# RayforceDB/rayforce

Hardware: AMD Instinct MI355X
Metric: rows/s on filter→group-by→sum, 1e9-row i64/f64; % HBM roofline at 1/2/4/8 GPU (higher is better)
Workload: dtype f64

## Files before the change

### include/rfx_hip.h

```cpp
#ifndef RFX_HIP_H
#define RFX_HIP_H

#ifndef __HIPCC_RTC__
#include <stddef.h>
#endif
#include <stdint.h>

#ifdef __cplusplus
extern "C" {
#endif
#ifndef __HIPCC_RTC__
#pragma GCC visibility push(default)
#endif

enum {
    RFX_OK = 0,
    RFX_ENODEV = -1,
    RFX_EINVAL = -2,
    RFX_ENOMEM = -3,
    RFX_EHIP = -4,
    RFX_ELIMIT = -5,
    RFX_ESTATE = -6
};

// ... 53 lines not shown
typedef struct rfx_xnode {
    int32_t op;
    int32_t _pad;
    rfx_xoperand_t l, r;
} rfx_xnode_t;

typedef struct rfx_agg {
    const void *d_col;
    int32_t col_type;
    int32_t kind;
    int32_t xop;
    int32_t xflags;
    const void *d_xrhs_col;
    int32_t xrhs_type;
    int32_t nxnodes;
    union {
        int64_t xrhs_i;
        double xrhs_f;
    };
    const rfx_xnode_t *xnodes;
} rfx_agg_t;
int rfx_agg_input_type(const rfx_agg_t *a);

typedef struct rfx_partial {
    int64_t isum;
    double fsum;
    int64_t cnt;
    int64_t ext;
    int64_t pos;
    int64_t _rsv[3];
} rfx_partial_t;

typedef struct rfx_value {
    int32_t type;
    int32_t is_null;
    union {
        int64_t i;
        double f;
    };
} rfx_value_t;

typedef struct rfx_ctx rfx_ctx_t;

int rfx_hip_device_count(void);
const char *rfx_hip_last_error(void);
const char *rfx_hip_version(void);
#define RFX_STREAM_LEGACY ((void *)(uintptr_t)1)
int rfx_hip_ctx_create(int device, void *stream, rfx_ctx_t **out);
int rfx_hip_ctx_destroy(rfx_ctx_t *ctx);
int rfx_hip_ctx_sync(rfx_ctx_t *ctx);
int rfx_hip_ctx_set_stream(rfx_ctx_t *ctx, void *stream);
enum {
    RFX_TUNE_NO_LDS_TABLES = 1,
    RFX_TUNE_NO_PARTITION = 2,
    RFX_TUNE_NO_BIG_LDS = 4,
    RFX_TUNE_PART_3WG = 8,
    RFX_TUNE_NO_WRITE_COMBINE = 16,
    RFX_TUNE_DIRECT_WC = 32,
    RFX_TUNE_FUSED_KEYS = 64,
    RFX_TUNE_NO_FUSED_SCOPE = 128,
    RFX_TUNE_NO_SOA_WC = 2048,
    RFX_TUNE_NO_LDS_SPLIT = 1024,
    RFX_TUNE_NO_EMIT_WC = 512,
    RFX_TUNE_NO_SEL_COMPACT = 256,
    RFX_TUNE_NO_DEEP_GROUP = 4096,
    RFX_TUNE_NO_LDS_REPLICAS = 8192,
    RFX_TUNE_NO_CHUNK = 16384,
    RFX_TUNE_CHUNK_SMALL = 32768,
    RFX_TUNE_CHUNK_CONTIG = 65536,
    RFX_TUNE_CHUNK_QUEUE = 131072,
    RFX_TUNE_CHUNK_BINS = 262144,
    RFX_TUNE_NO_RTC = 524288,
    RFX_TUNE_NO_PLANE = 1048576,
    RFX_TUNE_NO_WHERE_ONCE = 2097152
};
int rfx_hip_ctx_tune(rfx_ctx_t *ctx, int blocks_per_cu, int flags);
enum {
    RFX_STAT_PLANE_SCATTER = 0,
    RFX_STAT_PLANE_FALLBACK = 1,
    RFX_STAT_PLANE_AGGREGATE = 2,
    RFX_STAT_CHUNK_SCATTER = 3,
    RFX_STAT_CHUNK_AGGREGATE = 4,
    RFX_STAT_MASK_PASSES = 5,
    RFX_STAT_WHERE_ONCE = 6
};
int64_t rfx_hip_ctx_stat(rfx_ctx_t *ctx, int which);

int rfx_hip_malloc(rfx_ctx_t *ctx, void **d_ptr, size_t bytes);
int rfx_hip_free(rfx_ctx_t *ctx, void *d_ptr);
int rfx_hip_ctx_trim(rfx_ctx_t *ctx);
int rfx_hip_h2d(rfx_ctx_t *ctx, void *d_dst, const void *src, size_t bytes);
int rfx_hip_d2h(rfx_ctx_t *ctx, void *dst, const void *d_src, size_t bytes);
int rfx_hip_d2h_async(rfx_ctx_t *ctx, void *dst, const void *d_src, size_t bytes);
int rfx_hip_memset(rfx_ctx_t *ctx, void *d_dst, int byte, size_t bytes);
int rfx_hip_fill_i64(rfx_ctx_t *ctx, int64_t *d_dst, int64_t n, int64_t value);
void rfx_hip_rtc_stats(int64_t *launches, int64_t *compiles);
void rfx_hip_rtc_cache_stats(int64_t *loaded_from_disk, int64_t *written_to_disk);
int rfx_hip_rtc_prewarm_filter_aggr(const rfx_pred_t *preds, int npred, int logic, const rfx_agg_t *aggs, int nagg);
int rfx_hip_rtc_prewarm_where(const rfx_pred_t *preds, int npred, int logic);

int rfx_hip_h2d_pipelined(rfx_ctx_t *ctx, void *d_dst, const void *src, size_t bytes);
int rfx_hip_d2h_pipelined(rfx_ctx_t *ctx, void *dst, const void *d_src, size_t bytes);
int rfx_column_file_stat(const char *path, int32_t *type, int64_t *len);
int rfx_hip_column_file_load(rfx_ctx_t *ctx, const char *path, void *d_dst, int64_t nrows);
int rfx_hip_widen_i32(rfx_ctx_t *ctx, const int32_t *d_in, int64_t n, int64_t *d_out);
int rfx_hip_widen_b8(rfx_ctx_t *ctx, const int8_t *d_in, int64_t n, int64_t *d_out);

int rfx_hip_timer_start(rfx_ctx_t *ctx);
int rfx_hip_timer_stop(rfx_ctx_t *ctx, float *ms);
int rfx_hip_ctx_profile(rfx_ctx_t *ctx, int enable);
int rfx_hip_last_kernel_ms(rfx_ctx_t *ctx, float *ms);
int rfx_hip_profile_kernels(rfx_ctx_t *ctx, float *ms, int cap, int *n);

int rfx_hip_gen_i64(rfx_ctx_t *ctx, int64_t *d_out, int64_t n, uint64_t seed, int64_t row0, uint64_t modulus);
int rfx_hip_gen_f64(rfx_ctx_t *ctx, double *d_out, int64_t n, uint64_t seed, int64_t row0);

int rfx_hip_filter_aggr(rfx_ctx_t *ctx, const rfx_pred_t *preds, int npred, int logic, const rfx_agg_t *aggs,
                        int nagg, int64_t nrows, int64_t row0, rfx_partial_t *d_out);
void rfx_partial_merge(int kind, int col_type, rfx_partial_t *into, const rfx_partial_t *from);
void rfx_partial_identity(rfx_partial_t *p);
int rfx_agg_finalize(int kind, int col_type, const rfx_partial_t *p, rfx_value_t *out);
int rfx_hip_filter_aggr_host(rfx_ctx_t *ctx, const rfx_pred_t *preds, int npred, int logic, const rfx_agg_t *aggs,
                             int nagg, int64_t nrows, rfx_value_t *values, int64_t *selected);

int rfx_hip_cmp_mask(rfx_ctx_t *ctx, const rfx_pred_t *pred, int64_t nrows, int8_t *d_mask);
int rfx_hip_mask_logic(rfx_ctx_t *ctx, int logic, int8_t *d_acc, const int8_t *d_next, int scalar, int64_t nrows);

int rfx_hip_where_begin(rfx_ctx_t *ctx, const rfx_pred_t *preds, int npred, int logic, const int8_t *d_mask,
                        int64_t nrows, int64_t *count);
int rfx_hip_where_emit(rfx_ctx_t *ctx, int64_t row0, int64_t *d_ids);
int rfx_hip_where_estimate(rfx_ctx_t *ctx, const rfx_pred_t *preds, int npred, int logic, int64_t nrows, int64_t *upper);
int rfx_hip_where_once(rfx_ctx_t *ctx, const rfx_pred_t *preds, int npred, int logic, int64_t nrows, int64_t row0, int64_t *d_ids,
                       int64_t cap, int64_t *count);

int rfx_hip_gather(rfx_ctx_t *ctx, const void *d_col, const int64_t *d_ids, int64_t m, void *d_out);
int rfx_hip_gather_many(rfx_ctx_t *ctx, const void *const *d_cols, int ncols, const int64_t *d_ids, int64_t m, void *const *d_outs);
int rfx_hip_gather_checked(rfx_ctx_t *ctx, const void *d_col, int64_t col_len, int32_t col_type, const int64_t *d_ids, int64_t m, void *d_out);

int rfx_hip_scope_i64(rfx_ctx_t *ctx, const int64_t *d_key, const rfx_pred_t *preds, int npred, int logic,
                      int64_t nrows, int64_t *min, int64_t *max, int64_t *count);

int rfx_hip_group_scope(rfx_ctx_t *ctx, const int64_t *d_key, const rfx_pred_t *preds, int npred, int logic,
                        const rfx_agg_t *aggs, int nagg, int64_t nrows, int64_t *min, int64_t *max, int64_t *count);

typedef struct rfx_group_tables {
    int64_t kmin;
    int64_t range;
    int32_t nagg;
    int32_t _pad;
    int64_t *d_first;
    void *d_acc[RFX_MAX_AGGS];
    int64_t *d_cnt[RFX_MAX_AGGS];
} rfx_group_tables_t;

int rfx_hip_group_table_arrays(const rfx_agg_t *aggs, int nagg, int *n_arrays);
int rfx_hip_group_tables_init(rfx_ctx_t *ctx, const rfx_agg_t *aggs, const rfx_group_tables_t *t);
int rfx_hip_group_dense_accumulate(rfx_ctx_t *ctx, const int64_t *d_key, const rfx_pred_t *preds, int npred,
                                   int logic, const rfx_agg_t *aggs, int64_t nrows, int64_t row0,
                                   const rfx_group_tables_t *t);
int rfx_hip_group_rank(rfx_ctx_t *ctx, const rfx_group_tables_t *t, int64_t total_rows, int64_t *ngroups);
#define RFX_SCOPE_SAMPLE_ROWS (1 << 18)
#define RFX_SCOPE_SAMPLE_MAX_RANGE 16384
int rfx_hip_scope_sample_i64(rfx_ctx_t *ctx, const int64_t *d_key, int64_t nrows, int64_t *min, int64_t *max);
int rfx_hip_ctx_speculative(rfx_ctx_t *ctx, int on);
int rfx_hip_group_out_of_scope(rfx_ctx_t *ctx, int *violated);
#define RFX_RANK_SMALL 2048
int rfx_hip_group_rank_emit_small(rfx_ctx_t *ctx, const rfx_agg_t *aggs, const rfx_group_tables_t *t, int64_t row0, int64_t local_rows, int64_t *d_block);
int rfx_hip_group_emit(rfx_ctx_t *ctx, const rfx_agg_t *aggs, const rfx_group_tables_t *t, int64_t *d_keys,
                       int64_t *d_first_ids, void *const *d_results);
int rfx_hip_group_emit_sharded(rfx_ctx_t *ctx, const rfx_agg_t *aggs, const rfx_group_tables_t *t, int64_t row0, int64_t local_rows,
                               int64_t *d_keys, int64_t *d_first_ids, void *const *d_results);
#define RFX_RANK_EMIT_MAX (1 << 22)
#define RFX_SLICE_G0(g, i, nsl) ((int64_t)(i) * ((g) / (nsl)) + ((int64_t)(i) < (g) % (nsl) ? (int64_t)(i) : (g) % (nsl)))
#define RFX_SLICE_GN(g, i, nsl) ((g) / (nsl) + ((int64_t)(i) < (g) % (nsl) ? 1 : 0))
int rfx_hip_group_rank_emit(rfx_ctx_t *ctx, const rfx_agg_t *aggs, const rfx_group_tables_t *t, int64_t total_rows, int64_t row0, int64_t local_rows,
                            int nsl, int si, int64_t out_cap, int64_t *d_keys, int64_t *d_first_ids, void *const *d_results, int64_t *ngroups);
int rfx_hip_ctx_emit_window(rfx_ctx_t *ctx, int64_t g0, int64_t n);

typedef struct rfx_hash_tables {
    int64_t capacity;
    int32_t nagg;
    int32_t _pad;
    int64_t *d_keys;
    int64_t *d_first;
    void *d_acc[RFX_MAX_AGGS];
    int64_t *d_cnt[RFX_MAX_AGGS];
} rfx_hash_tables_t;
int rfx_hip_hash_tables_init(rfx_ctx_t *ctx, const rfx_agg_t *aggs, const rfx_hash_tables_t *t);
// ... 179 lines not shown
```

### include/rfx_ops.h

```cpp
#ifndef RFX_OPS_H
#define RFX_OPS_H

#include "rfx_abi.h"

#ifdef __cplusplus
extern "C" {
#endif
#ifndef __HIPCC_RTC__
#pragma GCC visibility push(default)
#endif

int rfx_host_bind(void);
int rfx_ops_set_device(int device);
int rfx_ops_set_shards(const int *devices, int ndevices, int nshards);
int rfx_ops_shards(void);
int rfx_ops_dist_init(int world, int rank, const void *id128);
int rfx_ops_dist_finalize(void);
struct rfx_exec;
struct rfx_exec *rfx_ops_exec(void);
const char *rfx_ops_last_error(void);

rfx_obj_p rfx_select(rfx_obj_p dict);

rfx_obj_p rfx_eq(rfx_obj_p x, rfx_obj_p y);
rfx_obj_p rfx_ne(rfx_obj_p x, rfx_obj_p y);
rfx_obj_p rfx_lt(rfx_obj_p x, rfx_obj_p y);
rfx_obj_p rfx_gt(rfx_obj_p x, rfx_obj_p y);
rfx_obj_p rfx_le(rfx_obj_p x, rfx_obj_p y);
rfx_obj_p rfx_ge(rfx_obj_p x, rfx_obj_p y);

rfx_obj_p rfx_add(rfx_obj_p x, rfx_obj_p y);
rfx_obj_p rfx_sub(rfx_obj_p x, rfx_obj_p y);
rfx_obj_p rfx_mul(rfx_obj_p x, rfx_obj_p y);
rfx_obj_p rfx_div(rfx_obj_p x, rfx_obj_p y);
rfx_obj_p rfx_floordiv(rfx_obj_p x, rfx_obj_p y);
rfx_obj_p rfx_mod(rfx_obj_p x, rfx_obj_p y);

rfx_obj_p rfx_left_join(rfx_obj_p *x, int64_t n);
rfx_obj_p rfx_inner_join(rfx_obj_p *x, int64_t n);

rfx_obj_p rfx_and(rfx_obj_p *x, int64_t n);
rfx_obj_p rfx_or(rfx_obj_p *x, int64_t n);
rfx_obj_p rfx_and_sf(rfx_obj_p *x, int64_t n);
rfx_obj_p rfx_or_sf(rfx_obj_p *x, int64_t n);
rfx_obj_p rfx_where(rfx_obj_p mask);
rfx_obj_p rfx_at(rfx_obj_p col, rfx_obj_p ids);

rfx_obj_p rfx_sum(rfx_obj_p x);
rfx_obj_p rfx_avg(rfx_obj_p x);
rfx_obj_p rfx_min(rfx_obj_p x);
rfx_obj_p rfx_max(rfx_obj_p x);
rfx_obj_p rfx_count(rfx_obj_p x);
rfx_obj_p rfx_first(rfx_obj_p x);
rfx_obj_p rfx_last(rfx_obj_p x);
rfx_obj_p rfx_dev(rfx_obj_p x);
rfx_obj_p rfx_med(rfx_obj_p x);
rfx_obj_p rfx_iasc(rfx_obj_p x);
rfx_obj_p rfx_idesc(rfx_obj_p x);
rfx_obj_p rfx_asc(rfx_obj_p x);
rfx_obj_p rfx_desc(rfx_obj_p x);
rfx_obj_p rfx_rank(rfx_obj_p x);
rfx_obj_p rfx_xasc(rfx_obj_p t, rfx_obj_p cols);
rfx_obj_p rfx_xdesc(rfx_obj_p t, rfx_obj_p cols);
int rfx_last_sort_on_gpu(void);
rfx_obj_p rfx_asof_join(rfx_obj_p *x, int64_t n);
rfx_obj_p rfx_bin(rfx_obj_p x, rfx_obj_p y);
rfx_obj_p rfx_binr(rfx_obj_p x, rfx_obj_p y);
int rfx_last_asof_on_gpu(void);
rfx_obj_p rfx_window_join(rfx_obj_p *x, int64_t n);
rfx_obj_p rfx_window_join1(rfx_obj_p *x, int64_t n);
int rfx_last_window_on_gpu(void);

rfx_obj_p rfx_distinct(rfx_obj_p x);
rfx_obj_p rfx_find(rfx_obj_p x, rfx_obj_p y);
rfx_obj_p rfx_in(rfx_obj_p x, rfx_obj_p y);
rfx_obj_p rfx_sect(rfx_obj_p x, rfx_obj_p y);
rfx_obj_p rfx_except(rfx_obj_p x, rfx_obj_p y);
rfx_obj_p rfx_union(rfx_obj_p x, rfx_obj_p y);
int rfx_last_set_on_gpu(void);
int rfx_last_set_route(void);
rfx_obj_p rfx_set_stats(rfx_obj_p ignored);

rfx_obj_p rfx_xrank(rfx_obj_p v, rfx_obj_p n);
rfx_obj_p rfx_xbar(rfx_obj_p x, rfx_obj_p y);
rfx_obj_p rfx_within(rfx_obj_p x, rfx_obj_p range);
rfx_obj_p rfx_floor(rfx_obj_p x);
rfx_obj_p rfx_ceil(rfx_obj_p x);
rfx_obj_p rfx_round(rfx_obj_p x);
rfx_obj_p rfx_neg(rfx_obj_p x);
int rfx_last_bucket_on_gpu(void);

rfx_obj_p rfx_update(rfx_obj_p update_dict);
rfx_obj_p rfx_group(rfx_obj_p keys);
rfx_obj_p rfx_pin(rfx_obj_p table_or_column);
rfx_obj_p rfx_unpin(rfx_obj_p table_or_column);
rfx_obj_p rfx_invalidate(rfx_obj_p table_or_column);
int rfx_ops_set_validation(int mode);
int rfx_ops_set_deterministic(int mode);
int rfx_ops_set_rank_slices(int on);
rfx_obj_p rfx_stats(rfx_obj_p ignored);
void rfx_cache_clear(void);
int64_t rfx_cache_bytes(void);
int rfx_last_select_on_gpu(void);

rfx_obj_p rfx_host_vector(int8_t type, int64_t len);
rfx_obj_p rfx_host_device_vector(int8_t type, int64_t len, const void *const *d_ptrs, int nptrs);
rfx_obj_p rfx_host_i64(int64_t v);
rfx_obj_p rfx_host_f64(double v);
rfx_obj_p rfx_host_symbol(const char *name);
rfx_obj_p rfx_host_list(int64_t len);
rfx_obj_p rfx_host_table(rfx_obj_p keys, rfx_obj_p vals);
rfx_obj_p rfx_host_dict(rfx_obj_p keys, rfx_obj_p vals);
rfx_obj_p rfx_host_fn(const char *name);
rfx_obj_p rfx_host_clone(rfx_obj_p o);
void rfx_host_drop(rfx_obj_p o);
int64_t rfx_host_intern(const char *s, int64_t len);
const char *rfx_host_symbol_name(int64_t id);
const char *rfx_host_error_text(rfx_obj_p err);

#ifndef __HIPCC_RTC__
#pragma GCC visibility pop
#endif
#ifdef __cplusplus
}
#endif
#endif
```

### rayforce_amd/_lib.py

```python
from __future__ import annotations

import ctypes as C
import os

RFX_OK = 0
RFX_ELIMIT = -5
RFX_ESTATE = -6
RFX_B8, RFX_I64, RFX_F64 = 1, 5, 10
RFX_I32 = 4
RFX_ROUND_FLOOR, RFX_ROUND_CEIL, RFX_ROUND_ROUND = 0, 1, 2
RFX_EQ, RFX_NE, RFX_LT, RFX_GT, RFX_LE, RFX_GE = range(6)
RFX_AND, RFX_OR = 0, 1
RFX_AGG_SUM, RFX_AGG_MIN, RFX_AGG_MAX, RFX_AGG_COUNT, RFX_AGG_AVG, RFX_AGG_FIRST, RFX_AGG_LAST = range(7)
RFX_MAX_PREDS = RFX_MAX_AGGS = RFX_MAX_COLS = RFX_MAX_KEYS = 8
RFX_RANK_SMALL = 2048
RFX_MAX_EXPRS = 4
NULL_I64 = -(2**63)
INF_I64 = 2**63 - 1

OPS = {"==": RFX_EQ, "!=": RFX_NE, "<": RFX_LT, ">": RFX_GT, "<=": RFX_LE, ">=": RFX_GE}
AGGS = {"sum": RFX_AGG_SUM, "min": RFX_AGG_MIN, "max": RFX_AGG_MAX, "count": RFX_AGG_COUNT, "avg": RFX_AGG_AVG,
        "first": RFX_AGG_FIRST, "last": RFX_AGG_LAST}


# ... 114 lines not shown


class Query(C.Structure):
    _fields_ = [("preds", C.POINTER(Pred)), ("npred", C.c_int32), ("logic", C.c_int32), ("d_mask", C.c_void_p), ("aggs", C.POINTER(Agg)),
                ("nagg", C.c_int32), ("nkeys", C.c_int32), ("d_keys", C.POINTER(C.c_void_p)), ("kxbar", C.POINTER(C.c_int64)), ("nrows", C.c_int64),
                ("cols", C.POINTER(QCol)), ("ncols", C.c_int32), ("flags", C.c_int32), ("key_scope", C.POINTER(C.c_int64)), ("row0", C.c_int64),
                ("d_sel_ids", C.POINTER(C.c_void_p)), ("sel_count", C.POINTER(C.c_int64))]


class Ids(C.Structure):
    _fields_ = [("nshards", C.c_int32), ("total", C.c_int64), ("count", C.c_int64 * RFX_MAX_SHARDS), ("d_ids", C.c_void_p * RFX_MAX_SHARDS)]


class GSlice(C.Structure):
    _fields_ = [("shard", C.c_int32), ("g0", C.c_int64), ("n", C.c_int64), ("d_keys", C.c_void_p), ("d_first", C.c_void_p),
                ("d_keycols", C.c_void_p * RFX_MAX_KEYS), ("d_results", C.c_void_p * RFX_EXEC_MAX_AGGS)]


_GROUPS_OWN = RFX_MAX_SHARDS * (4 + 2 * RFX_MAX_KEYS + RFX_EXEC_MAX_AGGS)


class Groups(C.Structure):
    _fields_ = [("groups", C.c_int64), ("path", C.c_int32), ("nkeys", C.c_int32), ("nagg", C.c_int32), ("d_keys", C.c_void_p),
                ("d_keycols", C.c_void_p * RFX_MAX_KEYS), ("d_first", C.c_void_p), ("d_results", C.c_void_p * RFX_EXEC_MAX_AGGS),
                ("result_type", C.c_int32 * RFX_EXEC_MAX_AGGS), ("d_probe", C.c_void_p), ("capacity", C.c_int64), ("d_block", C.c_void_p),
                ("h_block", C.c_void_p), ("block_bytes", C.c_size_t), ("own", C.c_void_p * _GROUPS_OWN), ("own_shard", C.c_int8 * _GROUPS_OWN), ("nown", C.c_int32),
                ("nslices", C.c_int32), ("slice", GSlice * RFX_MAX_SHARDS)]


TR_WORLD_RANK = C.CFUNCTYPE(C.c_int, C.c_void_p, C.POINTER(C.c_int), C.POINTER(C.c_int))
TR_ALLGATHER_HOST = C.CFUNCTYPE(C.c_int, C.c_void_p, C.c_void_p, C.c_size_t, C.c_void_p)
TR_ALLREDUCE = C.CFUNCTYPE(C.c_int, C.c_void_p, C.c_void_p, C.c_int64, C.c_int, C.c_int)
TR_ALLGATHER_DEV = C.CFUNCTYPE(C.c_int, C.c_void_p, C.c_void_p, C.c_size_t, C.c_void_p)


class Transport(C.Structure):
    _fields_ = [("user", C.c_void_p), ("world_rank", TR_WORLD_RANK), ("allgather_host", TR_ALLGATHER_HOST), ("allreduce", TR_ALLREDUCE),
                ("allgather_dev", TR_ALLGATHER_DEV)]


_P = C.POINTER
_ctx = C.c_void_p

PROTOTYPES = {
    "rfx_hip_device_count": (C.c_int, []),
    "rfx_hip_last_error": (C.c_char_p, []),
    "rfx_hip_version": (C.c_char_p, []),
    "rfx_hip_ctx_create": (C.c_int, [C.c_int, C.c_void_p, _P(_ctx)]),
    "rfx_hip_ctx_destroy": (C.c_int, [_ctx]),
    "rfx_hip_ctx_sync": (C.c_int, [_ctx]),
    "rfx_hip_ctx_set_stream": (C.c_int, [_ctx, C.c_void_p]),
    "rfx_hip_ctx_tune": (C.c_int, [_ctx, C.c_int, C.c_int]),
    "rfx_hip_ctx_stat": (C.c_int64, [_ctx, C.c_int]),
    "rfx_hip_malloc": (C.c_int, [_ctx, _P(C.c_void_p), C.c_size_t]),
    "rfx_hip_free": (C.c_int, [_ctx, C.c_void_p]),
    "rfx_hip_ctx_trim": (C.c_int, [_ctx]),
    "rfx_hip_h2d": (C.c_int, [_ctx, C.c_void_p, C.c_void_p, C.c_size_t]),
    "rfx_hip_d2h": (C.c_int, [_ctx, C.c_void_p, C.c_void_p, C.c_size_t]),
    "rfx_hip_d2h_async": (C.c_int, [_ctx, C.c_void_p, C.c_void_p, C.c_size_t]),
    "rfx_hip_d2h_pipelined": (C.c_int, [_ctx, C.c_void_p, C.c_void_p, C.c_size_t]),
    "rfx_hip_memset": (C.c_int, [_ctx, C.c_void_p, C.c_int, C.c_size_t]),
    "rfx_hip_fill_i64": (C.c_int, [_ctx, C.c_void_p, C.c_int64, C.c_int64]),
    "rfx_hip_rtc_stats": (None, [_P(C.c_int64), _P(C.c_int64)]),
    "rfx_hip_rtc_cache_stats": (None, [_P(C.c_int64), _P(C.c_int64)]),
    "rfx_hip_rtc_prewarm_filter_aggr": (C.c_int, [_P(Pred), C.c_int, C.c_int, _P(Agg), C.c_int]),
    "rfx_hip_rtc_prewarm_where": (C.c_int, [_P(Pred), C.c_int, C.c_int]),
    "rfx_hip_timer_start": (C.c_int, [_ctx]),
    "rfx_hip_timer_stop": (C.c_int, [_ctx, _P(C.c_float)]),
    "rfx_hip_ctx_profile": (C.c_int, [_ctx, C.c_int]),
    "rfx_hip_last_kernel_ms": (C.c_int, [_ctx, _P(C.c_float)]),
    "rfx_hip_profile_kernels": (C.c_int, [_ctx, _P(C.c_float), C.c_int, _P(C.c_int)]),
    "rfx_hip_gen_i64": (C.c_int, [_ctx, C.c_void_p, C.c_int64, C.c_uint64, C.c_int64, C.c_uint64]),
    "rfx_hip_gen_f64": (C.c_int, [_ctx, C.c_void_p, C.c_int64, C.c_uint64, C.c_int64]),
    "rfx_hip_filter_aggr": (C.c_int, [_ctx, _P(Pred), C.c_int, C.c_int, _P(Agg), C.c_int, C.c_int64, C.c_int64, C.c_void_p]),
    "rfx_partial_merge": (None, [C.c_int, C.c_int, _P(Partial), _P(Partial)]),
    "rfx_partial_identity": (None, [_P(Partial)]),
    "rfx_agg_finalize": (C.c_int, [C.c_int, C.c_int, _P(Partial), _P(Value)]),
    "rfx_hip_filter_aggr_host": (C.c_int, [_ctx, _P(Pred), C.c_int, C.c_int, _P(Agg), C.c_int, C.c_int64, _P(Value), _P(C.c_int64)]),
    "rfx_hip_cmp_mask": (C.c_int, [_ctx, _P(Pred), C.c_int64, C.c_void_p]),
    "rfx_hip_mask_logic": (C.c_int, [_ctx, C.c_int, C.c_void_p, C.c_void_p, C.c_int, C.c_int64]),
    "rfx_hip_where_begin": (C.c_int, [_ctx, _P(Pred), C.c_int, C.c_int, C.c_void_p, C.c_int64, _P(C.c_int64)]),
    "rfx_hip_where_emit": (C.c_int, [_ctx, C.c_int64, C.c_void_p]),
    "rfx_hip_widen_i32": (C.c_int, [_ctx, C.c_void_p, C.c_int64, C.c_void_p]),
    "rfx_hip_widen_b8": (C.c_int, [_ctx, C.c_void_p, C.c_int64, C.c_void_p]),
    "rfx_hip_where_estimate": (C.c_int, [_ctx, _P(Pred), C.c_int, C.c_int, C.c_int64, _P(C.c_int64)]),
    "rfx_hip_where_once": (C.c_int, [_ctx, _P(Pred), C.c_int, C.c_int, C.c_int64, C.c_int64, C.c_void_p, C.c_int64, _P(C.c_int64)]),
    "rfx_hip_gather": (C.c_int, [_ctx, C.c_void_p, C.c_void_p, C.c_int64, C.c_void_p]),
    "rfx_hip_gather_many": (C.c_int, [_ctx, _P(C.c_void_p), C.c_int, C.c_void_p, C.c_int64, _P(C.c_void_p)]),
    "rfx_hip_gather_checked": (C.c_int, [_ctx, C.c_void_p, C.c_int64, C.c_int32, C.c_void_p, C.c_int64, C.c_void_p]),
    "rfx_hip_scope_i64": (C.c_int, [_ctx, C.c_void_p, _P(Pred), C.c_int, C.c_int, C.c_int64, _P(C.c_int64), _P(C.c_int64), _P(C.c_int64)]),
    "rfx_hip_group_scope": (C.c_int, [_ctx, C.c_void_p, _P(Pred), C.c_int, C.c_int, _P(Agg), C.c_int, C.c_int64, _P(C.c_int64), _P(C.c_int64), _P(C.c_int64)]),
    "rfx_hip_group_table_arrays": (C.c_int, [_P(Agg), C.c_int, _P(C.c_int)]),
    "rfx_hip_group_tables_init": (C.c_int, [_ctx, _P(Agg), _P(GroupTables)]),
    "rfx_hip_group_dense_accumulate": (C.c_int, [_ctx, C.c_void_p, _P(Pred), C.c_int, C.c_int, _P(Agg), C.c_int64, C.c_int64, _P(GroupTables)]),
    "rfx_hip_group_rank": (C.c_int, [_ctx, _P(GroupTables), C.c_int64, _P(C.c_int64)]),
    "rfx_hip_group_emit": (C.c_int, [_ctx, _P(Agg), _P(GroupTables), C.c_void_p, C.c_void_p, _P(C.c_void_p)]),
    "rfx_hip_scope_sample_i64": (C.c_int, [_ctx, C.c_void_p, C.c_int64, _P(C.c_int64), _P(C.c_int64)]),
    "rfx_hip_ctx_speculative": (C.c_int, [_ctx, C.c_int]),
    "rfx_hip_ctx_emit_window": (C.c_int, [_ctx, C.c_int64, C.c_int64]),
    "rfx_hip_group_rank_emit": (C.c_int, [_ctx, _P(Agg), _P(GroupTables), C.c_int64, C.c_int64, C.c_int64, C.c_int, C.c_int, C.c_int64, C.c_void_p, C.c_void_p,
                                          _P(C.c_void_p), _P(C.c_int64)]),
    "rfx_hip_hash_rank_emit": (C.c_int, [_ctx, _P(Agg), _P(HashTables), C.c_int64, C.c_int64, C.c_int64, C.c_int, C.c_int, C.c_int64, C.c_void_p, C.c_void_p,
                                         _P(C.c_void_p), _P(C.c_int64)]),
    "rfx_hip_group_out_of_scope": (C.c_int, [_ctx, _P(C.c_int)]),
    "rfx_hip_group_rank_emit_small": (C.c_int, [_ctx, _P(Agg), _P(GroupTables), C.c_int64, C.c_int64, C.c_void_p]),
    "rfx_hip_group_emit_sharded": (C.c_int, [_ctx, _P(Agg), _P(GroupTables), C.c_int64, C.c_int64, C.c_void_p, C.c_void_p, _P(C.c_void_p)]),
    "rfx_hip_hash_emit_sharded": (C.c_int, [_ctx, _P(Agg), _P(HashTables), C.c_int64, C.c_int64, C.c_void_p, C.c_void_p, _P(C.c_void_p)]),
    "rfx_hip_hash_tables_init": (C.c_int, [_ctx, _P(Agg), _P(HashTables)]),
    "rfx_hip_group_hash_accumulate": (C.c_int, [_ctx, C.c_void_p, _P(Pred), C.c_int, C.c_int, _P(Agg), C.c_int64, C.c_int64, _P(HashTables)]),
    "rfx_hip_group_hash_accumulate_slots": (C.c_int, [_ctx, C.c_void_p, _P(Pred), C.c_int, C.c_int, _P(Agg), C.c_int64, C.c_int64, _P(HashTables), C.c_void_p, _P(C.c_int)]),
    "rfx_hip_hash_slot_first": (C.c_int, [_ctx, _P(HashTables), C.c_void_p, C.c_int64, C.c_void_p]),
    "rfx_hip_hash_tables_init_packed": (C.c_int, [_ctx, _P(Agg), _P(HashTables), C.c_int]),
    "rfx_hip_group_hash_accumulate_packed": (C.c_int, [_ctx, C.c_void_p, _P(Pred), C.c_int, C.c_int, _P(Agg), C.c_int64, C.c_int64, _P(HashTables), C.c_int, C.c_void_p]),
    "rfx_hip_hash_tables_merge": (C.c_int, [_ctx, _P(Agg), _P(HashTables), _P(HashTables)]),
    "rfx_hip_hash_rank": (C.c_int, [_ctx, _P(HashTables), C.c_int64, _P(C.c_int64)]),
    "rfx_hip_hash_emit": (C.c_int, [_ctx, _P(Agg), _P(HashTables), C.c_void_p, C.c_void_p, _P(C.c_void_p)]),
    "rfx_hip_group_slot_ids": (C.c_int, [_ctx, _P(GroupTables), C.c_void_p]),
    "rfx_hip_group_ids_dense": (C.c_int, [_ctx, C.c_void_p, C.c_int64, _P(GroupTables), C.c_void_p]),
    "rfx_hip_group_ids_table": (C.c_int, [_ctx, C.c_void_p, C.c_int64, C.c_int64, C.c_int64, C.c_void_p, C.c_void_p]),
    "rfx_hip_group_ids_first": (C.c_int, [_ctx, C.c_void_p, C.c_int64, C.c_void_p, C.c_int64, C.c_void_p]),
    "rfx_hip_update_set": (C.c_int, [_ctx, C.c_void_p, C.c_void_p, C.c_int64, C.c_void_p, C.c_uint64]),
    "rfx_hip_update_select": (C.c_int, [_ctx, C.c_void_p, C.c_void_p, C.c_uint64, C.c_void_p, C.c_void_p, C.c_uint64, C.c_int64]),
    "rfx_hip_absmax_f64": (C.c_int, [_ctx, C.c_void_p, C.c_int64, _P(C.c_double), _P(C.c_int)]),
    "rfx_hip_fix_f64": (C.c_int, [_ctx, C.c_void_p, C.c_int64, C.c_int, C.c_void_p]),
    "rfx_hip_fix_f64_low": (C.c_int, [_ctx, C.c_void_p, C.c_int64, C.c_int, C.c_int, C.c_void_p]),
    "rfx_hip_unfix_f64": (C.c_int, [_ctx, C.c_void_p, C.c_void_p, C.c_void_p, C.c_int64, C.c_double, C.c_double]),
    "rfx_hip_update_group": (C.c_int, [_ctx, C.c_void_p, C.c_void_p, C.c_void_p, C.c_int64, _P(Agg), _P(GroupTables)]),
    "rfx_dist_unique_id": (C.c_int, [C.c_void_p]),
    "rfx_dist_init": (C.c_int, [_ctx, C.c_int, C.c_int, C.c_void_p]),
    "rfx_dist_finalize": (C.c_int, [_ctx]),
    "rfx_dist_world": (C.c_int, [_ctx, _P(C.c_int), _P(C.c_int)]),
    "rfx_dist_scope": (C.c_int, [_ctx, _P(C.c_int64), _P(C.c_int64), _P(C.c_int64)]),
    "rfx_dist_group_tables_allreduce": (C.c_int, [_ctx, _P(Agg), _P(GroupTables)]),
    "rfx_dist_partials_allgather": (C.c_int, [_ctx, C.c_void_p, C.c_int, C.c_void_p]),
    "rfx_dist_filter_aggr_host": (C.c_int, [_ctx, _P(Pred), C.c_int, C.c_int, _P(Agg), C.c_int, C.c_int64, C.c_int64, _P(Value), _P(C.c_int64)]),
    "rfx_dist_allreduce_i64": (C.c_int, [_ctx, C.c_void_p, C.c_int64, C.c_int]),
    "rfx_dist_allgather": (C.c_int, [_ctx, C.c_void_p, C.c_size_t, C.c_void_p]),
    "rfx_dist_calls": (C.c_int64, [_ctx]),
    "rfx_hip_hash_fnv1a_i64": (C.c_int, [_ctx, C.c_void_p, C.c_int64, C.c_void_p]),
    "rfx_hip_hash_mix_u64": (C.c_int, [_ctx, C.c_void_p, C.c_int64, C.c_uint64, C.c_void_p]),
    "rfx_agg_input_type": (C.c_int, [_P(Agg)]),
    "rfx_hip_xbar_i64": (C.c_int, [_ctx, C.c_void_p, C.c_int64, C.c_int64, C.c_void_p]),
    "rfx_hip_group_median": (C.c_int, [_ctx, _P(MedRows), C.c_void_p, C.c_int32, C.c_int64, C.c_int64, C.c_int32, C.c_void_p]),
    "rfx_hip_median": (C.c_int, [_ctx, C.c_void_p, C.c_int, C.c_int, C.c_void_p, C.c_void_p, C.c_int64, _P(Value)]),
    "rfx_hip_median_keys": (C.c_int, [_ctx, C.c_void_p, C.c_int32, C.c_int64, C.c_void_p]),
    "rfx_hip_last_rows": (C.c_int, [_ctx, C.c_void_p, C.c_int32, C.c_int64, C.c_int64, C.c_void_p]),
    "rfx_hip_last_gather": (C.c_int, [_ctx, _P(C.c_void_p), _P(C.c_int64), _P(C.c_int64), C.c_int, C.c_int32, C.c_void_p, C.c_int64, C.c_void_p]),
    "rfx_hip_dev_derive": (C.c_int, [_ctx, C.c_void_p, C.c_int32, C.c_int64, C.c_void_p, C.c_void_p]),
    "rfx_hip_dev_finalise": (C.c_int, [_ctx, C.c_void_p, C.c_void_p, C.c_void_p, C.c_int64, C.c_void_p]),
    "rfx_hip_dev": (C.c_int, [_ctx, C.c_void_p, C.c_int32, C.c_int64, _P(Value)]),
    "rfx_hip_key_slot_table": (C.c_int, [_ctx, C.c_void_p, C.c_int64, C.c_int64, C.c_int64, C.c_void_p]),
    "rfx_hip_sort_index": (C.c_int, [_ctx, C.c_void_p, C.c_int32, C.c_int64, C.c_int, C.c_void_p, C.c_void_p, _P(C.c_int32)]),
    "rfx_hip_sort_values": (C.c_int, [_ctx, C.c_void_p, C.c_int32, C.c_int64, C.c_int, C.c_void_p, C.c_void_p, _P(C.c_int32)]),
    "rfx_hip_inverse_perm": (C.c_int, [_ctx, C.c_void_p, C.c_int64, C.c_void_p]),
    "rfx_hip_xrank": (C.c_int, [_ctx, C.c_void_p, C.c_int64, C.c_int64, C.c_void_p]),
    "rfx_hip_xrank_sorted": (C.c_int, [_ctx, C.c_int64, C.c_int64, C.c_int, C.c_void_p]),
    "rfx_hip_xbar": (C.c_int, [_ctx, _P(XbarDesc), C.c_int64, C.c_void_p]),
    "rfx_hip_round_f64": (C.c_int, [_ctx, C.c_int, C.c_void_p, C.c_int64, C.c_void_p]),
    "rfx_hip_neg": (C.c_int, [_ctx, C.c_int32, C.c_void_p, C.c_int64, C.c_void_p]),
    "rfx_hip_within_i64": (C.c_int, [_ctx, C.c_void_p, C.c_int64, C.c_int64, C.c_int64, C.c_void_p]),
    "rfx_hip_seg_search": (C.c_int, [_ctx, C.c_void_p, C.c_int64, C.c_void_p, C.c_int64, C.c_void_p, C.c_int64, C.c_void_p, C.c_void_p, C.c_int, C.c_int64, C.c_void_p]),
    "rfx_hip_asof_runs": (C.c_int, [_ctx, C.c_void_p, C.c_int64, C.c_void_p]),
    "rfx_hip_set_scope": (C.c_int, [_ctx, C.c_void_p, C.c_int64, C.c_void_p, C.c_int64, _P(C.c_int64)]),
    "rfx_hip_set_mark": (C.c_int, [_ctx, C.c_void_p, C.c_int64, C.c_void_p, C.c_int64, C.c_int64, C.c_int64, C.c_void_p]),
    "rfx_hip_set_first_dense": (C.c_int, [_ctx, C.c_void_p, C.c_int64, C.c_int64, C.c_int64, C.c_void_p]),
    "rfx_hip_set_hash_build": (C.c_int, [_ctx, C.c_void_p, C.c_int64, C.c_void_p, C.c_int64, C.c_void_p, C.c_void_p, C.c_int64]),
# ... 126 lines not shown
```

### rayforce_amd/csrc/rfx_ctx.hip

```cpp
#include <pthread.h>
#include "rfx_common.hpp"
#include <stdarg.h>
#include <stdlib.h>

static thread_local char g_err[512] = "";

void rfx_set_error(const char *fmt, ...) {
    va_list ap;
    va_start(ap, fmt);
    vsnprintf(g_err, sizeof(g_err), fmt, ap);
    va_end(ap);
}

extern "C" const char *rfx_hip_last_error(void) { return g_err; }
extern "C" const char *rfx_hip_version(void) { return "rfx-hip 0.1 (gfx950)"; }

extern "C" int rfx_hip_device_count(void) {
    int n = 0;
    if (hipGetDeviceCount(&n) != hipSuccess) return 0;
    return n;
}

extern "C" int rfx_hip_ctx_create(int device, void *stream, rfx_ctx_t **out) {
    RFX_REQUIRE(out != NULL, RFX_EINVAL, "out is NULL");
    int n = 0;
    if (hipGetDeviceCount(&n) != hipSuccess || n <= 0) {
        rfx_set_error("no HIP device visible (hipGetDeviceCount failed or returned 0) -- the MI355X path has no CPU fallback");
        return RFX_ENODEV;
    }
    RFX_REQUIRE(device >= 0 && device < n, RFX_EINVAL, "device ordinal out of range");
    RFX_HIP_CHECK(hipSetDevice(device));
    hipDeviceProp_t prop;
    RFX_HIP_CHECK(hipGetDeviceProperties(&prop, device));
    rfx_ctx *c = (rfx_ctx *)calloc(1, sizeof(rfx_ctx));
    RFX_REQUIRE(c != NULL, RFX_ENOMEM, "host calloc failed");
    c->device = device;
    c->ext_p[7] = calloc(1, sizeof(CtxExt));
    RFX_REQUIRE(c->ext_p[7] != NULL, RFX_ENOMEM, "host calloc failed");
    c->num_cus = prop.multiProcessorCount > 0 ? prop.multiProcessorCount : 256;
    c->blocks_per_cu = 2;
    if (stream) {
        c->stream = (stream == RFX_STREAM_LEGACY) ? (hipStream_t)0 : (hipStream_t)stream;
        c->own_stream = false;
    } else {
        RFX_HIP_CHECK(hipStreamCreateWithFlags(&c->stream, hipStreamNonBlocking));
        c->own_stream = true;
    }
    RFX_HIP_CHECK(hipEventCreate(&c->ev0));
    RFX_HIP_CHECK(hipEventCreate(&c->ev1));
    for (int i = 0; i < 8; i++) {
        RFX_HIP_CHECK(hipEventCreate(&c->evk[i][0]));
        RFX_HIP_CHECK(hipEventCreate(&c->evk[i][1]));
    }
    c->pin_bytes = 1 << 16;
    RFX_HIP_CHECK(hipHostMalloc(&c->h_pin, c->pin_bytes, hipHostMallocDefault));
    int rc = rfx_ws_reserve(c, 4u << 20);
    if (rc != RFX_OK) return rc;
    *out = c;
    return RFX_OK;
}

static void pool_release(rfx_ctx *c);
void rfx_plane_release(rfx_ctx *c);
void rfx_plane_invalidate(rfx_ctx *c);
extern "C" int rfx_hip_ctx_destroy(rfx_ctx_t *c) {
    if (!c) return RFX_OK;
    (void)hipSetDevice(c->device);
    (void)hipStreamSynchronize(c->stream);
    (void)rfx_dist_finalize(c);
    if (c->d_dist) (void)hipFree(c->d_dist);
    if (c->d_ws) (void)hipFree(c->d_ws);
    if (c->d_bitmap) (void)hipFree(c->d_bitmap);
    if (c->d_blksum) (void)hipFree(c->d_blksum);
    if (c->d_gid) (void)hipFree(c->d_gid);
    if (c->d_part) (void)hipFree(c->d_part);
    if (c->d_comp) (void)hipFree(c->d_comp);
    if (c->d_sel) (void)hipFree(c->d_sel);
    if (c->d_expr) (void)hipFree(c->d_expr);
    if (c->d_chunk) (void)hipFree(c->d_chunk);
    rfx_io_release(c);
    pool_release(c);
    if (c->ext_p[1]) (void)hipFree(c->ext_p[1]);
    free(c->ext_p[7]);
    free(c->ext_p[5]);
    free(c->ext_p[6]);
    rfx_plane_release(c);
    if (c->d_pc_counts) (void)hipFree(c->d_pc_counts);
    if (c->h_pin) (void)hipHostFree(c->h_pin);
    (void)hipEventDestroy(c->ev0);
    (void)hipEventDestroy(c->ev1);
    for (int i = 0; i < 8; i++) {
        (void)hipEventDestroy(c->evk[i][0]);
        (void)hipEventDestroy(c->evk[i][1]);
    }
    if (c->own_stream) (void)hipStreamDestroy(c->stream);
    free(c);
    return RFX_OK;
}

extern "C" int64_t rfx_hip_ctx_stat(rfx_ctx_t *c, int which) {
    if (!c || which < 0 || which > 6) return -1;
    if (which == 6) return (int64_t)(uintptr_t)c->ext_p[4];
    return which == RFX_STAT_MASK_PASSES ? c->ext_i[0] : c->ext_i[3 + which];
}

extern "C" int rfx_hip_ctx_sync(rfx_ctx_t *c) {
    RFX_REQUIRE(c, RFX_EINVAL, "ctx is NULL");
    RFX_HIP_CHECK(hipStreamSynchronize(c->stream));
    return RFX_OK;
}

extern "C" int rfx_hip_ctx_set_stream(rfx_ctx_t *c, void *stream) {
    RFX_REQUIRE(c, RFX_EINVAL, "ctx is NULL");
    RFX_REQUIRE(stream, RFX_EINVAL, "stream is NULL");
    if (c->own_stream) {
        (void)hipStreamSynchronize(c->stream);
        (void)hipStreamDestroy(c->stream);
        c->own_stream = false;
    }
    c->stream = (stream == RFX_STREAM_LEGACY) ? (hipStream_t)0 : (hipStream_t)stream;
    return RFX_OK;
}

extern "C" int rfx_hip_ctx_tune(rfx_ctx_t *c, int blocks_per_cu, int flags) {
    RFX_REQUIRE(c, RFX_EINVAL, "ctx is NULL");
    if (blocks_per_cu > 0) {
        RFX_REQUIRE(blocks_per_cu <= 64, RFX_EINVAL, "blocks_per_cu > 64");
        c->blocks_per_cu = blocks_per_cu;
    }
    c->flags = flags;
    return RFX_OK;
}

int rfx_ws_reserve(rfx_ctx *c, size_t bytes) {
    if (c->ws_bytes >= bytes) return RFX_OK;
    RFX_HIP_CHECK(hipStreamSynchronize(c->stream));
    if (c->d_ws) RFX_HIP_CHECK(hipFree(c->d_ws));
    c->d_ws = NULL;
    c->ws_bytes = 0;
    RFX_HIP_CHECK(hipMalloc(&c->d_ws, bytes));
    c->ws_bytes = bytes;
    return RFX_OK;
}

int rfx_bitmap_reserve(rfx_ctx *c, i64 nrows) {
    size_t words = (size_t)((nrows + 63) / 64) + 64;
    size_t blocks = (size_t)((nrows + 2047) / 2048) + 2;
    if (c->bitmap_cap < words) {
        RFX_HIP_CHECK(hipStreamSynchronize(c->stream));
        if (c->d_bitmap) RFX_HIP_CHECK(hipFree(c->d_bitmap));
        c->d_bitmap = NULL;
        c->bitmap_cap = 0;
        RFX_HIP_CHECK(hipMalloc((void **)&c->d_bitmap, words * 8));
        c->bitmap_cap = words;
    }
    if (c->blksum_cap < blocks) {
        RFX_HIP_CHECK(hipStreamSynchronize(c->stream));
        if (c->d_blksum) RFX_HIP_CHECK(hipFree(c->d_blksum));
        c->d_blksum = NULL;
        c->blksum_cap = 0;
        RFX_HIP_CHECK(hipMalloc((void **)&c->d_blksum, blocks * 8));
        c->blksum_cap = blocks;
    }
    return RFX_OK;
}

int rfx_gid_reserve(rfx_ctx *c, i64 slots) {
    if (c->gid_cap >= (size_t)slots) return RFX_OK;
    RFX_HIP_CHECK(hipStreamSynchronize(c->stream));
    if (c->d_gid) RFX_HIP_CHECK(hipFree(c->d_gid));
    c->d_gid = NULL;
    c->gid_cap = 0;
    RFX_HIP_CHECK(hipMalloc((void **)&c->d_gid, (size_t)slots * 8));
    c->gid_cap = (size_t)slots;
    return RFX_OK;
}

int rfx_part_reserve(rfx_ctx *c, size_t bytes) {
    if (c->part_bytes >= bytes) return RFX_OK;
    RFX_HIP_CHECK(hipStreamSynchronize(c->stream));
    if (c->d_part) RFX_HIP_CHECK(hipFree(c->d_part));
    c->d_part = NULL;
    c->part_bytes = 0;
    RFX_HIP_CHECK(hipMalloc(&c->d_part, bytes));
// ... 617 lines not shown
```

### rayforce_amd/csrc/rfx_group_plane.hip

```cpp
#include "rfx_part_common.hpp"
#include <stdlib.h>

#define PL_T 1024
#define PL_WAVES (PL_T / RFX_WAVE)
#define PL_WROWS 512
#define PL_BLOCK_ROWS (1 << 18)
#define PL_DELTA_BITS 18
#define PL_SLOT_BITS 14
#define PL_QCAP 320
#define PL_QFLUSH 24
#define PL_SPIN_LIMIT (1u << 14)
#define PL_MAX_NV 3
#ifndef PL_META64_PLAIN
#define PL_META64_PLAIN 1
#endif

struct PlaneArgs {
    int nblk;
    int nv;
    unsigned pmask;
    i64 block_rows;
    unsigned c0;
    u64 *vals[PL_MAX_NV];
    unsigned *meta;
    unsigned *cnt;
    unsigned *ctl;
};
struct PlSh {
    unsigned dead, _pad[3];
    i64 red[3][PL_WAVES];
};
template <int PBITS, int VGL, bool HK>
__host__ __device__ constexpr int pl_parts() { return (HK && PBITS == 8 && VGL == 4) ? 192 : (1 << PBITS); }
template <int NV, int PBITS, int VGL, bool HK = false>
__host__ __device__ constexpr size_t pl_lds_bytes() {
    return (size_t)pl_parts<PBITS, VGL, HK>() * ((size_t)(2 << VGL) * (NV * 8 + 4) + 8 + 4) + (size_t)PL_WAVES * PL_QCAP * 4 + sizeof(PlSh) + 64;
}
typedef u64 pl_v2 __attribute__((ext_vector_type(2)));
typedef unsigned pl_m2 __attribute__((ext_vector_type(2)));
#define PL_LD(ptr) __hip_atomic_load((ptr), __ATOMIC_RELAXED, __HIP_MEMORY_SCOPE_WORKGROUP)
#define PL_ST(ptr, v) __hip_atomic_store((ptr), (v), __ATOMIC_RELAXED, __HIP_MEMORY_SCOPE_WORKGROUP)

template <int NC, int NP, int NV, int PBITS, int VGL, bool HK = false>
__global__ __launch_bounds__(PL_T) void k_plane_scatter(const Plan P, const PlaneArgs A) {
    constexpr int PARTS = pl_parts<PBITS, VGL, HK>();
    constexpr bool P192 = PARTS != (1 << PBITS);
    constexpr unsigned VG = 1u << VGL, RING = 2u << VGL;
    constexpr bool KVI = HK && NV == 2 && PBITS == 8 && VGL == 3;
    constexpr unsigned LPD = VG / 2;
    extern __shared__ __attribute__((aligned(16))) unsigned char pl_smem[];
    u64 *vring = (u64 *)pl_smem;
    unsigned *mring = (unsigned *)(vring + (size_t)NV * PARTS * RING);
    unsigned *words = mring + (size_t)PARTS * RING;
    unsigned *tail = words + PARTS * 2;
    unsigned *fq = tail + PARTS;
    PlSh &L = *(PlSh *)(fq + PL_WAVES * PL_QCAP);
    PredSet<NP> S;
    predset_load<NP>(P, S);
    const int tid = threadIdx.x, lane = tid & 63, wv = tid >> 6;
    unsigned *myq = fq + wv * PL_QCAP;
    const i64 r0 = (i64)blockIdx.x * A.block_rows;
    const i64 r1 = (r0 + A.block_rows < P.nrows) ? r0 + A.block_rows : P.nrows;
    const u64 region = ((u64)blockIdx.x * (u64)PARTS) * A.c0;
    for (int i = tid; i < PARTS; i += PL_T) {
        tail[i] = 0;
        words[2 * i] = 0;
        words[2 * i + 1] = 0;
    }
    if (tid == 0) L.dead = 0;
    __syncthreads();
    i64 mn = RFX_INF_I64_D, mx = RFX_NULL_I64_D;
    unsigned nsel = 0;
    int qn = 0;

    auto flush_queue = [&]() __attribute__((always_inline)) {
        asm volatile("" ::: "memory");
        for (int i0 = 0; i0 < qn; i0 += 64 / (int)LPD) {
            const int idx = i0 + (lane / (int)LPD);
            if (idx < qn) {
                const unsigned d = myq[idx];
                const unsigned p = d & 0xFFu, gi = (d >> 8) & 0x3FFFFFu, pl = d >> 30, sub = lane & (LPD - 1u);
                if (pl < 3) {
                    const pl_v2 x = *(const pl_v2 *)(vring + ((size_t)pl * PARTS + p) * RING + (gi & 1u) * VG + sub * 2);
                    if constexpr (KVI) {
                        __builtin_nontemporal_store(x, (pl_v2 *)(A.vals[0] + 2 * (region + (u64)p * A.c0 + (u64)gi * VG) + (u64)pl * VG + sub * 2));
                    } else {
                        u64 *dst = (NV == 1 ? A.vals[0] : (pl == 0 ? A.vals[0] : (pl == 1 ? A.vals[1] : A.vals[2])));
                        __builtin_nontemporal_store(x, (pl_v2 *)(dst + region + (u64)p * A.c0 + (u64)gi * VG + sub * 2));
                    }
                } else if (sub < LPD / 2) {
                    const pl_v2 x = *(const pl_v2 *)(mring + (size_t)p * RING + (gi & 1u) * VG + sub * 4);
                    if constexpr (KVI || (VGL == 4 && PL_META64_PLAIN)) *(pl_v2 *)(A.meta + region + (u64)p * A.c0 + (u64)gi * VG + sub * 4) = x;
                    else __builtin_nontemporal_store(x, (pl_v2 *)(A.meta + region + (u64)p * A.c0 + (u64)gi * VG + sub * 4));
                }
            }
        }
        asm volatile("" ::: "memory");
        for (int i = lane; i < qn; i += 64) {
            const unsigned d = myq[i];
            if ((d >> 30) == 3u) atomicAdd(&words[2 * (d & 0xFFu) + ((d >> 8) & 1u)], 256u - VG);
        }
        qn = 0;
    };

    auto place = [&](const bool on, const u64 key, const u64 (&val)[NV], const unsigned delta) __attribute__((always_inline)) {
        const u64 kh = HK ? rfx_hash_index_u64(RFX_U64_HASH_SEED, key) : key;
        const unsigned p = P192 ? (unsigned)(((kh >> 32) * (u64)PARTS) >> 32) : (HK ? (unsigned)(kh >> (64 - PBITS)) : ((unsigned)key & (unsigned)(PARTS - 1)));
        unsigned seq = 0;
        if (on) {
            const i64 k = (i64)key;
            mn = k < mn ? k : mn;
            mx = k > mx ? k : mx;
            seq = atomicAdd(&tail[p], 1u);
            if (seq >= A.c0) PL_ST(&L.dead, 1u);
        }
        const unsigned g = seq >> VGL;
        unsigned *w = &words[2 * p + (g & 1u)];
        bool todo = on && seq < A.c0;
        for (unsigned it = 0;; it++) {
            bool ready = false;
            if (todo) ready = (PL_LD(w) >> 8) == (g >> 1);
            bool comp = false;
            if (ready) {
                const unsigned at = p * RING + (seq & (RING - 1u));
#pragma unroll
                for (int j = 0; j < NV; j++) vring[(size_t)j * PARTS * RING + at] = val[j];
                mring[at] = ((unsigned)(P192 ? (kh >> 18) : (HK ? (kh >> (64 - PBITS - PL_SLOT_BITS)) : (key >> PBITS))) & ((1u << PL_SLOT_BITS) - 1u)) | (delta << PL_SLOT_BITS);
                asm volatile("" ::: "memory");
                comp = (atomicAdd(w, 1u) & 0xFFu) == VG - 1u;
                todo = false;
            }
            const u64 cb = __ballot(comp);
            if (cb) {
                if (comp) {
                    const unsigned at = (unsigned)qn + (unsigned)(NV + 1) * __builtin_amdgcn_mbcnt_hi((unsigned)(cb >> 32), __builtin_amdgcn_mbcnt_lo((unsigned)cb, 0u));
#pragma unroll
                    for (int j = 0; j < NV; j++) myq[at + j] = p | (g << 8) | ((unsigned)j << 30);
                    myq[at + NV] = p | (g << 8) | (3u << 30);
                }
                qn += (NV + 1) * __popcll(cb);
            }
            if (!__any(todo)) break;
            flush_queue();
            if (PL_LD(&L.dead) || it > PL_SPIN_LIMIT) {
                PL_ST(&L.dead, 1u);
                break;
            }
            if (it) __builtin_amdgcn_s_sleep(4);
        }
        if (qn >= PL_QFLUSH) flush_queue();
    };

    bool alive = true;
    auto step = [&](const u64 (&v)[NC][8], const unsigned m, const i64 sbase) __attribute__((always_inline)) {
        const unsigned dbase = (unsigned)(sbase - r0);
        const unsigned valid = m;
        if constexpr (NP == 0) {
            nsel += (unsigned)__popc(valid);
#pragma unroll
            for (int e = 0; e < 8; e++) {
                u64 val[NV];
#pragma unroll
                for (int j = 0; j < NV; j++) val[j] = v[1 + j][e];
                place((valid >> e) & 1u, v[0][e], val, dbase + (unsigned)((e >> 1) * 128 + (e & 1)));
            }
        } else {
            unsigned rem = m;
            nsel += (unsigned)__popc(rem);
            u64 t[1 + NV][8];
#pragma unroll
            for (int c = 0; c < 1 + NV; c++) {
#pragma unroll
                for (int q = 0; q < 8; q++) {
                    t[c][q] = v[c][q];
                    if constexpr (NV > 1) asm volatile("" : "+v"(t[c][q]));
                }
            }
            while (__any(rem != 0u)) {
                const bool on = rem != 0u;
                const unsigned e = (unsigned)__builtin_ctz(rem | 0x100u);
                rem &= rem - 1u;
                u64 key = t[0][0], val[NV];
#pragma unroll
                for (int j = 0; j < NV; j++) val[j] = t[1 + j][0];
#pragma unroll
                for (int q = 1; q < 8; q++) {
                    const bool is = e == (unsigned)q;
                    key = is ? t[0][q] : key;
#pragma unroll
                    for (int j = 0; j < NV; j++) val[j] = is ? t[1 + j][q] : val[j];
                }
                place(on, key, val, dbase + (e >> 1) * 128u + (e & 1u));
            }
        }
        flush_queue();
        if (PL_LD(&L.dead)) alive = false;
    };

    const i64 nsteps = (r1 - r0 + PL_WROWS - 1) / PL_WROWS;
    const i64 nfull = (r1 - r0) / PL_WROWS;
    {
        u64 va[NC][8];
        for (i64 s = wv; s < nfull && alive; s += PL_WAVES) {
            const i64 base = r0 + s * PL_WROWS + lane * 2;
            if constexpr (NP == 0) {
#pragma unroll
                for (int c = 0; c < NC; c++) {
#pragma unroll
                    for (int j = 0; j < 4; j++) {
                        const u64x2 t = rfx_ld2(P.cols[c] + base + j * 128);
                        va[c][2 * j] = t.x;
                        va[c][2 * j + 1] = t.y;
                    }
                }
                step(va, 0xffu, base);
            } else {
#pragma unroll
                for (int c = 0; c < NC; c++) {
                    if ((A.pmask >> c) & 1u) {
#pragma unroll
                        for (int j = 0; j < 4; j++) {
                            const u64x2 t = rfx_ld2(P.cols[c] + base + j * 128);
                            va[c][2 * j] = t.x;
                            va[c][2 * j + 1] = t.y;
                        }
                    } else {
#pragma unroll
                        for (int e = 0; e < 8; e++) va[c][e] = 0;
                    }
                }
                const unsigned m = eval_preds<NC, 8, NP>(S, va, 0xffu);
#pragma unroll
                for (int c = 0; c < NC; c++) {
                    if (!((A.pmask >> c) & 1u)) {
#pragma unroll
                        for (int j = 0; j < 4; j++) {
                            if ((m >> (2 * j)) & 3u) {
                                const u64x2 t = rfx_ld2(P.cols[c] + base + j * 128);
                                va[c][2 * j] = t.x;
                                va[c][2 * j + 1] = t.y;
                            }
                        }
                    }
                }
                step(va, m, base);
            }
        }
    }
    if (nfull < nsteps && (nfull % PL_WAVES) == wv && alive) {
        u64 va[NC][8];
        const i64 base = r0 + nfull * PL_WROWS + lane * 2;
        unsigned valid = 0;
#pragma unroll
        for (int e = 0; e < 8; e++) {
            const i64 row = base + (e >> 1) * 128 + (e & 1);
            const bool in = row < r1;
            valid |= (unsigned)in << e;
#pragma unroll
            for (int c = 0; c < NC; c++) va[c][e] = in ? P.cols[c][row] : 0ULL;
        }
        step(va, (NP == 0) ? valid : eval_preds<NC, 8, NP>(S, va, valid), base);
    }
    __syncthreads();
    if (L.dead) {
        if (tid == 0) atomicExch(&A.ctl[1], 1u);
        return;
    }
    for (int i = tid; i < PARTS * (NV + 1) * (int)LPD; i += PL_T) {
        const unsigned sub = (unsigned)i & (LPD - 1u), p = ((unsigned)i / LPD) % (unsigned)PARTS, pl = ((unsigned)i / LPD) / (unsigned)PARTS;
        const unsigned t = tail[p];
        if (!(t & (VG - 1u))) continue;
        const unsigned gi = t >> VGL;
        if (pl < (unsigned)NV) {
            const pl_v2 x = *(const pl_v2 *)(vring + ((size_t)pl * PARTS + p) * RING + (gi & 1u) * VG + sub * 2);
            if constexpr (KVI) {
                *(pl_v2 *)(A.vals[0] + 2 * (region + (u64)p * A.c0 + (u64)gi * VG) + (u64)pl * VG + sub * 2) = x;
            } else {
                u64 *dst = (NV == 1 ? A.vals[0] : (pl == 0 ? A.vals[0] : (pl == 1 ? A.vals[1] : A.vals[2])));
                *(pl_v2 *)(dst + region + (u64)p * A.c0 + (u64)gi * VG + sub * 2) = x;
            }
        } else if (sub < LPD / 2) {
            const pl_v2 x = *(const pl_v2 *)(mring + (size_t)p * RING + (gi & 1u) * VG + sub * 4);
            *(pl_v2 *)(A.meta + region + (u64)p * A.c0 + (u64)gi * VG + sub * 4) = x;
        }
    }
    for (int i = tid; i < PARTS; i += PL_T) A.cnt[(size_t)blockIdx.x * PARTS + i] = tail[i];
    i64 sel = (i64)nsel;
    for (int s2 = 32; s2 >= 1; s2 >>= 1) {
        const i64 omn = (i64)rfx_shfl_xor_u64((u64)mn, s2), omx = (i64)rfx_shfl_xor_u64((u64)mx, s2);
        mn = omn < mn ? omn : mn;
        mx = omx > mx ? omx : mx;
        sel += (i64)rfx_shfl_xor_u64((u64)sel, s2);
    }
    if (lane == 0) {
        L.red[0][wv] = mn;
        L.red[1][wv] = mx;
        L.red[2][wv] = sel;
    }
    __syncthreads();
    if (tid == 0) {
        for (int w2 = 1; w2 < PL_WAVES; w2++) {
            mn = L.red[0][w2] < mn ? L.red[0][w2] : mn;
            mx = L.red[1][w2] > mx ? L.red[1][w2] : mx;
            sel += L.red[2][w2];
        }
        unsigned long long *g = (unsigned long long *)A.ctl + 8;
        if (sel > 0) {
            atomicMax(&g[0], ~((unsigned long long)mn ^ 0x8000000000000000ULL));
            atomicMax(&g[1], (unsigned long long)mx ^ 0x8000000000000000ULL);
            atomicAdd(&g[2], (unsigned long long)sel);
        }
    }
}

struct PlaneAggArgs {
    i64 kmin, range;
    i64 local;
    int split;
    int excl;
    int first_read;
    int nblk, pbits;
    int agg_pl[RFX_MAX_AGGS];
    i64 block_rows;
    unsigned c0;
    const u64 *vals[PL_MAX_NV];
    const unsigned *meta;
    const unsigned *cnt;
    u64 *first;
    u64 *acc[RFX_MAX_AGGS];
    u64 *cntt[RFX_MAX_AGGS];
};
#define PL_FIRST_NONE 0xFFFFFFFFu

template <int THREADS, int NVL, bool FAST>
__global__ __launch_bounds__(THREADS) void k_plane_aggregate(const Plan P, const PlaneAggArgs A) {
    extern __shared__ __attribute__((aligned(16))) u64 pl_agg_smem[];
    const int tid = threadIdx.x;
    const int p = blockIdx.x / A.split, s = blockIdx.x % A.split;
    const i64 local = A.local;
    int kind[RFX_MAX_AGGS], f64[RFX_MAX_AGGS], skip[RFX_MAX_AGGS], cnt_of[RFX_MAX_AGGS], apl[RFX_MAX_AGGS];
    int ncnt = 0;
#pragma unroll
// ... 84 lines not shown
        }
    };
    const int q = __builtin_amdgcn_readfirstlane(s * NW + (tid >> 6));
    const int nreg = q < A.nblk ? (A.nblk - q + Q - 1) / Q : 0;
    unsigned *wcnt = cnts + (i64)ncnt * local + (tid >> 6) * 64;
    int r = -1;
    int b = q;
    unsigned i0 = 0, n = 0;
    auto advance = [&]() __attribute__((always_inline)) {
        for (;;) {
            if (r >= 0 && i0 < n) return true;
            r++;
            if (r >= nreg) return false;
            if ((r & 63) == 0) {
                const int r0 = r + lane;
                wcnt[lane] = (r0 < nreg) ? A.cnt[((size_t)(q + r0 * Q) << A.pbits) + p] : 0u;
            }
            n = (unsigned)__builtin_amdgcn_readfirstlane((int)wcnt[r & 63]);
            b = q + r * Q;
            i0 = 0;
        }
    };
    Batch B0, B1;
    bool h0 = advance();
    load(h0, b, i0, n, B0);
    i0 += 256u;
    while (h0) {
        const bool h1 = advance();
        load(h1, b, i0, n, B1);
        i0 += 256u;
        consume(B0);
        if (!h1) break;
        h0 = advance();
        load(h0, b, i0, n, B0);
        i0 += 256u;
        consume(B1);
    }
    __syncthreads();
    for (i64 i = tid; i < local; i += THREADS) {
        const unsigned f = first[i];
        if (f == PL_FIRST_NONE) continue;
        const i64 g = (i << A.pbits) | (i64)(((u64)p - (u64)A.kmin) & (u64)((1 << A.pbits) - 1));
        if (g >= A.range) continue;
        const u64 fr = (u64)P.row0 + (u64)f;
        if (A.excl) {
            if (fr < A.first[g]) A.first[g] = fr;
#pragma unroll
            for (int a = 0; a < RFX_MAX_AGGS; a++) {
                if (kind[a] < 0) continue;
                const bool hc = cnt_of[a] >= 0;
                group_merge_cell_plain(&A.acc[a][g], hc ? &A.cntt[a][g] : (u64 *)0, kind[a], f64[a], accs[(i64)a * local + i], hc ? (u64)cnts[(i64)cnt_of[a] * local + i] : 0ULL);
            }
            continue;
        }
        if (fr < A.first[g]) atomicMin((unsigned long long *)&A.first[g], (unsigned long long)fr);
#pragma unroll
        for (int a = 0; a < RFX_MAX_AGGS; a++) {
            if (kind[a] < 0) continue;
            const bool hc = cnt_of[a] >= 0;
            group_merge_cell(&A.acc[a][g], hc ? &A.cntt[a][g] : (u64 *)0, kind[a], f64[a], accs[(i64)a * local + i], hc ? (u64)cnts[(i64)cnt_of[a] * local + i] : 0ULL);
        }
    }
}

int rfx_chunk_reserve(rfx_ctx *c, size_t bytes);
static size_t pl_al256(size_t x) { return (x + 255) & ~(size_t)255; }

static void plane_layout(rfx_ctx *c, int nblk, int pbits, unsigned c0, int nv, PlaneArgs *A, size_t *total, int parts = 0) {
    const size_t regions = parts ? (size_t)nblk * (size_t)parts : (size_t)nblk << pbits;
    const size_t o_cnt = 256;
    const size_t o_meta = o_cnt + pl_al256(regions * 4), o_val = o_meta + pl_al256(regions * c0 * 4);
    const size_t plane = pl_al256(regions * c0 * 8);
    if (total) *total = o_val + plane * nv;
    char *w = (char *)c->d_chunk;
    A->nblk = nblk;
    A->nv = nv;
    A->c0 = c0;
    A->ctl = (unsigned *)w;
    A->cnt = (unsigned *)(w + o_cnt);
    A->meta = (unsigned *)(w + o_meta);
    for (int j = 0; j < nv; j++) A->vals[j] = (u64 *)(w + o_val + plane * j);
}

template <int NC, int NP, int NV, int PBITS, int VGL, bool HK = false>
static int launch_plane_scatter_inst(rfx_ctx *c, const Plan &P, const PlaneArgs &A) {
    constexpr size_t lds = pl_lds_bytes<NV, PBITS, VGL, HK>();
    static_assert(lds <= 160 * 1024, "rings beyond a CU's LDS");
    static unsigned long long attr_set = 0;
    if (!((attr_set >> (c->device & 63)) & 1ull)) {
        RFX_HIP_CHECK(hipFuncSetAttribute((const void *)k_plane_scatter<NC, NP, NV, PBITS, VGL, HK>, hipFuncAttributeMaxDynamicSharedMemorySize, (int)lds));
        __atomic_fetch_or(&attr_set, 1ull << (c->device & 63), __ATOMIC_RELAXED);
    }
    hipLaunchKernelGGL((k_plane_scatter<NC, NP, NV, PBITS, VGL, HK>), dim3(A.nblk), dim3(PL_T), lds, c->stream, P, A);
    return RFX_OK;
}
template <int NC, int NV, int PBITS, int VGL, bool HK = false>
static int launch_plane_scatter_np(rfx_ctx *c, const Plan &P, const PlaneArgs &A) {
    if (P.npred == 0) return launch_plane_scatter_inst<NC, 0, NV, PBITS, VGL, HK>(c, P, A);
    if (P.npred == 1) return launch_plane_scatter_inst<NC, 1, NV, PBITS, VGL, HK>(c, P, A);
    if (P.npred <= 3) return launch_plane_scatter_inst<NC, 3, NV, PBITS, VGL, HK>(c, P, A);
    return launch_plane_scatter_inst<NC, RFX_MAX_PREDS, NV, PBITS, VGL, HK>(c, P, A);
}
static int launch_plane_scatter(rfx_ctx *c, const Plan &P, const PlaneArgs &A, int pbits) {
    const int extra = P.ncols - 1 - A.nv;
    if (extra < 0 || extra > 2) return RFX_ESTATE;
    if (A.nv == 1) {
        if (pbits == 7) return extra == 0 ? launch_plane_scatter_np<2, 1, 7, 5>(c, P, A) : (extra == 1 ? launch_plane_scatter_np<3, 1, 7, 5>(c, P, A) : launch_plane_scatter_np<4, 1, 7, 5>(c, P, A));
        return extra == 0 ? launch_plane_scatter_np<2, 1, 8, 4>(c, P, A) : (extra == 1 ? launch_plane_scatter_np<3, 1, 8, 4>(c, P, A) : launch_plane_scatter_np<4, 1, 8, 4>(c, P, A));
    }
    if (pbits != 7 || extra > 1) return RFX_ESTATE;
    if (A.nv == 2) return extra == 0 ? launch_plane_scatter_np<3, 2, 7, 4>(c, P, A) : launch_plane_scatter_np<4, 2, 7, 4>(c, P, A);
    return extra == 0 ? launch_plane_scatter_np<4, 3, 7, 4>(c, P, A) : launch_plane_scatter_np<5, 3, 7, 4>(c, P, A);
}

static int plane_value_cols(const Plan &P, int *vcol, int *agg_plane) {
    int nv = 0;
    for (int a = 0; a < P.nagg; a++) {
        const PlanAgg &ag = P.aggs[a];
        agg_plane[a] = -1;
        if (ag.kind == RFX_AGG_COUNT || ag.kind == RFX_AGG_FIRST || ag.col < 0) continue;
        if (ag.col >= RFX_XCOL) return -1;
        int j = 0;
        for (; j < nv; j++)
            if (vcol[j] == ag.col) break;
        if (j == nv) {
            if (nv >= PL_MAX_NV) return -1;
            vcol[nv++] = ag.col;
        }
        agg_plane[a] = j;
    }
    return nv;
}
static size_t plane_agg_lds(const Plan &P, int a0, int a1, i64 local) {
    size_t cells8 = 0, cells4 = 1;
    for (int a = a0; a < a1; a++) {
        cells8++;
        if (agg_has_cnt(P.aggs[a].kind, P.aggs[a].f64)) cells4++;
    }
    return (size_t)local * (cells8 * 8 + cells4 * 4) + 16 * 64 * 4 + 64;
}
#define PL_AGG_LDS_MAX (150 * 1024)
static bool plane_agg_fits(const Plan &P, i64 local) {
    for (int a = 0; a < P.nagg; a++)
        if (plane_agg_lds(P, a, a + 1, local) > PL_AGG_LDS_MAX) return false;
    return P.nagg >= 1;
}

struct PlaneState {
    int valid, npred, logic, nblk, pbits, nv;
    unsigned c0;
    const void *key;
    const void *val[PL_MAX_NV];
    i64 nrows;
    i64 seen;
    u64 sig[RFX_MAX_PREDS][6];
};
static PlaneState *plane_state(rfx_ctx *c) {
    if (!c->ext_p[2]) c->ext_p[2] = calloc(1, sizeof(PlaneState));
    return (PlaneState *)c->ext_p[2];
}
void rfx_plane_invalidate(rfx_ctx *c) {
    if (c->ext_p[2]) ((PlaneState *)c->ext_p[2])->valid = 0;
}
void rfx_plane_release(rfx_ctx *c) {
    free(c->ext_p[2]);
    c->ext_p[2] = NULL;
}
static void plane_pred_sig(const Plan &P, u64 (*sig)[6]) {
    for (int i = 0; i < P.npred; i++) {
        const PlanPred &q = P.preds[i];
        sig[i][0] = (u64)(uintptr_t)P.cols[q.col];
        sig[i][1] = q.rhs_col >= 0 ? (u64)(uintptr_t)P.cols[q.rhs_col] : 0;
        sig[i][2] = (u64)q.op;
        sig[i][3] = (u64)(q.dom_f64 | (q.lhs_cvt << 1) | (q.rhs_cvt << 2) | (q.more << 3) | ((u64)q.tree << 4));
        sig[i][4] = q.rhs_bits;
        sig[i][5] = 0;
    }
}

int rfx_plane_scope(rfx_ctx *c, const Plan &P, int key_idx, const void *d_key, int npred, int logic, unsigned long long est_range, double frac,
                    i64 *kmin, i64 *kmax, i64 *seen) {
    PlaneState *st = plane_state(c);
    if (!st) return RFX_ESTATE;
    st->valid = 0;
    if (c->flags & RFX_TUNE_NO_PLANE) return RFX_ESTATE;
    int vcol[PL_MAX_NV], agg_plane[RFX_MAX_AGGS];
    const int nv = plane_value_cols(P, vcol, agg_plane);
    if (nv < 1 || P.nx > 0) return RFX_ESTATE;
    int pbits = 7;
    {
        static const char *force = getenv("RFX_PLANE_PBITS");
        const i64 l7 = (i64)((est_range + 127) >> 7);
        if (l7 + l7 / 16 > (1 << PL_SLOT_BITS) || !plane_agg_fits(P, l7 + l7 / 16)) pbits = 8;
        if (force && nv == 1) pbits = atoi(force) == 7 ? 7 : 8;
    }
    if (pbits == 8 && nv > 1) return RFX_ESTATE;
    const i64 est_local = (i64)((est_range + (1ULL << pbits) - 1) >> pbits);
    if (est_local > (1 << PL_SLOT_BITS) || !plane_agg_fits(P, est_local)) return RFX_ESTATE;
    const i64 nrows = P.nrows;
    const i64 nblk64 = (nrows + PL_BLOCK_ROWS - 1) / PL_BLOCK_ROWS;
    if (nblk64 > (1 << 20) || nrows >= 0xFFFFFFF0LL) return RFX_ESTATE;
    double share = (double)PL_BLOCK_ROWS / (double)(1 << pbits);
    if (npred > 0) share *= (frac * 1.3 + 0.01 < 1.0 ? frac * 1.3 + 0.01 : 1.0);
    unsigned c0 = (unsigned)(share * 1.25 + 160.0);
    c0 = (c0 + 127u) & ~127u;
    PlaneArgs A;
    memset(&A, 0, sizeof(A));
    size_t need = 0;
    plane_layout(c, (int)nblk64, pbits, c0, nv, &A, &need);
    if (rfx_chunk_reserve(c, need) != RFX_OK) return RFX_ESTATE;
    plane_layout(c, (int)nblk64, pbits, c0, nv, &A, NULL);
    A.block_rows = PL_BLOCK_ROWS;
    Plan Pc = P;
    {
        int perm[RFX_MAX_COLS + PL_MAX_NV], inv[RFX_MAX_COLS], n2 = 0;
        for (int i = 0; i < P.ncols; i++) inv[i] = -1;
        perm[n2++] = key_idx;
        inv[key_idx] = 0;
        for (int j = 0; j < nv; j++) {
            if (inv[vcol[j]] < 0) inv[vcol[j]] = n2;
            perm[n2++] = vcol[j];
        }
        for (int i = 0; i < P.ncols; i++)
            if (inv[i] < 0) {
                inv[i] = n2;
                perm[n2++] = i;
            }
        if (n2 > 1 + nv + 2 || n2 > RFX_MAX_COLS) return RFX_ESTATE;
        Pc.ncols = n2;
        for (int i = 0; i < n2; i++) Pc.cols[i] = P.cols[perm[i]];
        for (int i = 0; i < P.npred; i++) {
            Pc.preds[i].col = inv[P.preds[i].col];
            if (P.preds[i].rhs_col >= 0) Pc.preds[i].rhs_col = inv[P.preds[i].rhs_col];
        }
    }
    for (int i = 0; i < Pc.npred; i++) {
        A.pmask |= 1u << Pc.preds[i].col;
        if (Pc.preds[i].rhs_col >= 0) A.pmask |= 1u << Pc.preds[i].rhs_col;
    }
    if (getenv("RFX_PLANE_LOAD_ALL")) A.pmask = 0xFFu;
    RFX_HIP_CHECK(hipMemsetAsync(A.ctl, 0, 256, c->stream));
    c->ext_i[3 + RFX_STAT_PLANE_SCATTER]++;
    RFX_KERNEL_BEGIN(c);
    int rc = launch_plane_scatter(c, Pc, A, pbits);
    RFX_KERNEL_END(c);
    if (rc != RFX_OK) return rc;
    RFX_HIP_CHECK(hipGetLastError());
    unsigned *hctl = (unsigned *)c->h_pin;
    RFX_HIP_CHECK(hipMemcpyAsync(hctl, A.ctl, 256, hipMemcpyDeviceToHost, c->stream));
    RFX_HIP_CHECK(hipStreamSynchronize(c->stream));
    if (hctl[1]) {
        c->ext_i[3 + RFX_STAT_PLANE_FALLBACK]++;
        return RFX_ESTATE;
    }
    const u64 *hs = (const u64 *)hctl + 8;
    *seen = (i64)hs[2];
    plane_state(c)->seen = *seen;
    *kmin = (i64)(~hs[0] ^ 0x8000000000000000ULL);
    *kmax = (i64)(hs[1] ^ 0x8000000000000000ULL);
    if (*seen > 0 && *kmin == RFX_NULL_I64_D) return RFX_ESTATE;
    if (*seen == 0) return RFX_OK;
    st->valid = 1;
    st->key = d_key;
    for (int j = 0; j < nv; j++) st->val[j] = (const void *)P.cols[vcol[j]];
    st->nrows = nrows;
    st->npred = npred;
    st->logic = logic;
    st->nblk = (int)nblk64;
    st->pbits = pbits;
    st->nv = nv;
    st->c0 = c0;
    plane_pred_sig(P, st->sig);
    return RFX_OK;
}

template <int THREADS, int NVL, bool FAST>
static int launch_plane_aggregate_inst(rfx_ctx *c, const Plan &P, const PlaneAggArgs &G, int grid, size_t lds, int lds_max) {
    static unsigned long long attr_set = 0;
    if (!((attr_set >> (c->device & 63)) & 1ull)) {
        RFX_HIP_CHECK(hipFuncSetAttribute((const void *)k_plane_aggregate<THREADS, NVL, FAST>, hipFuncAttributeMaxDynamicSharedMemorySize, lds_max));
        __atomic_fetch_or(&attr_set, 1ull << (c->device & 63), __ATOMIC_RELAXED);
    }
    hipLaunchKernelGGL((k_plane_aggregate<THREADS, NVL, FAST>), dim3(grid), dim3(THREADS), lds, c->stream, P, G);
    return RFX_OK;
}
template <int THREADS>
static int launch_plane_aggregate(rfx_ctx *c, const Plan &P, const PlaneAggArgs &G, int nvl, bool fast, int grid, size_t lds, int lds_max) {
    if (nvl <= 1) return fast ? launch_plane_aggregate_inst<THREADS, 1, true>(c, P, G, grid, lds, lds_max) : launch_plane_aggregate_inst<THREADS, 1, false>(c, P, G, grid, lds, lds_max);
    if (nvl == 2) return launch_plane_aggregate_inst<THREADS, 2, false>(c, P, G, grid, lds, lds_max);
    return launch_plane_aggregate_inst<THREADS, 3, false>(c, P, G, grid, lds, lds_max);
}

int rfx_plane_accumulate(rfx_ctx *c, const Plan &P, int key_idx, const rfx_group_tables_t *t) {
    PlaneState *st = (PlaneState *)c->ext_p[2];
    if (!st || !st->valid) return RFX_ESTATE;
    int vcol[PL_MAX_NV], agg_plane[RFX_MAX_AGGS];
    bool ok = st->key == (const void *)P.cols[key_idx] && st->nrows == P.nrows && st->npred == P.npred && st->logic == P.logic && P.nx == 0;
    const int nv = ok ? plane_value_cols(P, vcol, agg_plane) : -1;
    ok = ok && nv == st->nv;
    for (int j = 0; ok && j < nv; j++) ok = st->val[j] == (const void *)P.cols[vcol[j]];
    if (ok && P.npred > 0) {
        u64 sig[RFX_MAX_PREDS][6];
        plane_pred_sig(P, sig);
        ok = memcmp(sig, st->sig, sizeof(u64) * 6 * (size_t)P.npred) == 0;
    }
    st->valid = 0;
    if (!ok || t->range <= (1 << st->pbits)) return RFX_ESTATE;
    const i64 local = (t->range + (1 << st->pbits) - 1) >> st->pbits;
    if (local > (1 << PL_SLOT_BITS) || !plane_agg_fits(P, local)) return RFX_ESTATE;
    PlaneArgs A;
    memset(&A, 0, sizeof(A));
    plane_layout(c, st->nblk, st->pbits, st->c0, st->nv, &A, NULL);
    const int nparts = 1 << st->pbits;
    RFX_KERNEL_BEGIN(c);
    int rc = RFX_OK;
    for (int a0 = 0; a0 < P.nagg && rc == RFX_OK;) {
        int a1 = a0 + 1;
        while (a1 < P.nagg && plane_agg_lds(P, a0, a1 + 1, local) <= PL_AGG_LDS_MAX) a1++;
        Plan Ps = P;
        Ps.nagg = a1 - a0;
        PlaneAggArgs G;
        memset(&G, 0, sizeof(G));
        G.kmin = t->kmin;
        G.range = t->range;
        G.local = local;
        {
            static const char *fr = getenv("RFX_PL_FIRST_READ");
            G.first_read = fr ? atoi(fr) : 1;
        }
// ... 547 lines not shown
```

### rayforce_amd/csrc/rfx_io.hip

```cpp
#include <errno.h>
#include <fcntl.h>
#include <pthread.h>
#include <sys/mman.h>
#include <sys/stat.h>
#include <unistd.h>
#include "rfx_common.hpp"

#define IO_CHUNK ((size_t)32 << 20)
#define IO_NBUF 4
#define IO_PIECE ((size_t)2 << 20)
#define IO_MAX_WORKERS 64
#define IO_QUEUE 4096

struct IoJob {
    char *dst;
    const char *src;
    size_t bytes;
    int fd;
    int *left;
};
static struct {
    pthread_mutex_t mu;
    pthread_cond_t cv_work, cv_done;
    IoJob q[IO_QUEUE];
// ... 200 lines not shown
}

struct ColHeader {
    uint8_t mmod, order;
    int8_t type;
    uint8_t attrs;
    uint32_t rc;
    int64_t len;
};
static_assert(sizeof(ColHeader) == 16, "column file header");

static int elem_size(int type) {
    switch (type) {
        case 5:
        case 6:
        case 9:
        case 10:
            return 8;
        default: return 0;
    }
}

extern "C" int rfx_column_file_stat(const char *path, int32_t *type, int64_t *len) {
    RFX_REQUIRE(path && type && len, RFX_EINVAL, "NULL argument");
    int fd = open(path, O_RDONLY);
    if (fd < 0) {
        rfx_set_error("rfx_column_file_stat: cannot open %s", path);
        return RFX_EINVAL;
    }
    ColHeader h;
    struct stat st;
    const bool ok = read(fd, &h, sizeof(h)) == (ssize_t)sizeof(h) && fstat(fd, &st) == 0;
    close(fd);
    if (!ok || h.mmod != 0xfd) {
        rfx_set_error("rfx_column_file_stat: %s is not a RayforceDB column file (16-byte header with mmod 0xfd expected)", path);
        return RFX_EINVAL;
    }
    const int es = elem_size(h.type);
    if (!es) {
        rfx_set_error("rfx_column_file_stat: %s holds type %d; only 8-byte columns (i64 / symbol ids / timestamp / f64) are on this path", path, (int)h.type);
        return RFX_EINVAL;
    }
    if (h.len < 0 || st.st_size < 16 || h.len > ((int64_t)st.st_size - 16) / es) {
        rfx_set_error("rfx_column_file_stat: %s is truncated (%lld rows declared)", path, (long long)h.len);
        return RFX_EINVAL;
    }
    *type = h.type;
    *len = h.len;
    return RFX_OK;
}

extern "C" int rfx_hip_column_file_load(rfx_ctx_t *c, const char *path, void *d_dst, int64_t nrows) {
    RFX_REQUIRE(c && path, RFX_EINVAL, "NULL argument");
    int32_t type;
    int64_t len;
    int rc = rfx_column_file_stat(path, &type, &len);
    if (rc != RFX_OK) return rc;
    RFX_REQUIRE(nrows == len, RFX_EINVAL, "nrows does not match the file's length");
    if (len == 0) return RFX_OK;
    RFX_REQUIRE(d_dst != NULL, RFX_EINVAL, "d_dst is NULL");
    int fd = open(path, O_RDONLY);
    RFX_REQUIRE(fd >= 0, RFX_EINVAL, "cannot open the column file");
    const size_t bytes = (size_t)len * 8;
    if (bytes < IO_CHUNK) {
        void *tmp = malloc(bytes);
        if (!tmp) {
            close(fd);
            return RFX_ENOMEM;
        }
        io_read_here((char *)tmp, (const char *)(size_t)16, bytes, fd);
        rc = rfx_hip_h2d(c, d_dst, tmp, bytes);
        free(tmp);
    } else rc = h2d_pipelined_from(c, d_dst, (const void *)(size_t)16, bytes, fd);
    close(fd);
    return rc;
}

__global__ __launch_bounds__(256) void k_widen_i32(const int32_t *__restrict__ in, long long n, long long *__restrict__ out) {
    for (long long i = blockIdx.x * 256LL + threadIdx.x; i < n; i += (long long)gridDim.x * 256LL) {
        const int32_t x = in[i];
        out[i] = x == (int32_t)0x80000000 ? (long long)0x8000000000000000ULL : (long long)x;
    }
}
__global__ __launch_bounds__(256) void k_widen_b8(const int8_t *__restrict__ in, long long n, long long *__restrict__ out) {
    for (long long i = blockIdx.x * 256LL + threadIdx.x; i < n; i += (long long)gridDim.x * 256LL) out[i] = in[i] ? 1LL : 0LL;
}
extern "C" int rfx_hip_widen_b8(rfx_ctx_t *c, const int8_t *d_in, int64_t n, int64_t *d_out) {
    RFX_REQUIRE(c, RFX_EINVAL, "ctx is NULL");
    if (n <= 0) return RFX_OK;
    RFX_REQUIRE(d_in && d_out, RFX_EINVAL, "NULL argument");
    long long blocks = (n + 255) / 256;
    int grid = c->num_cus * 16;
    if (blocks < grid) grid = (int)blocks;
    hipLaunchKernelGGL(k_widen_b8, dim3(grid), dim3(256), 0, c->stream, d_in, (long long)n, (long long *)d_out);
    RFX_HIP_CHECK(hipGetLastError());
    return RFX_OK;
}
extern "C" int rfx_hip_widen_i32(rfx_ctx_t *c, const int32_t *d_in, int64_t n, int64_t *d_out) {
    RFX_REQUIRE(c, RFX_EINVAL, "ctx is NULL");
    if (n <= 0) return RFX_OK;
    RFX_REQUIRE(d_in && d_out, RFX_EINVAL, "NULL argument");
    long long blocks = (n + 255) / 256;
    int grid = c->num_cus * 16;
    if (blocks < grid) grid = (int)blocks;
    hipLaunchKernelGGL(k_widen_i32, dim3(grid), dim3(256), 0, c->stream, d_in, (long long)n, (long long *)d_out);
    RFX_HIP_CHECK(hipGetLastError());
    return RFX_OK;
}
```

### rayforce_amd/csrc/rfx_ops.c

```c
#define _GNU_SOURCE
#include <dlfcn.h>
#include <stdint.h>
#include <stdio.h>
#include <pthread.h>
#include <stdlib.h>
#include <unistd.h>
#include <fcntl.h>
#include <sys/mman.h>
#include <string.h>
#include <math.h>
#include <time.h>
#include "rfx_abi.h"
#include "rfx_hip.h"
#include "rfx_exec.h"
#include "rfx_ops.h"

typedef rfx_obj_p obj_p;

obj_p rfx_host_null(void);
obj_p rfx_host_b8(int8_t v);
obj_p rfx_host_err(const char *msg);
obj_p rfx_host_eval(obj_p o);
void rfx_host_trim(void);

// ... 63 lines not shown
        g_host_where = dlsym(RTLD_DEFAULT, "ray_where");
        g_host_at = dlsym(RTLD_DEFAULT, "ray_at");
        g_host_group = dlsym(RTLD_DEFAULT, "ray_group");
        if (H.i64 && H.f64 && H.drop && H.clone && H.err && H.intern && H.symname) {
            H.bound = 1;
            return 1;
        }
    }
    H.vector = rfx_host_vector;
    H.table = rfx_host_table;
    H.i64 = rfx_host_i64;
    H.f64 = rfx_host_f64;
    H.drop = rfx_host_drop;
    H.clone = rfx_host_clone;
    H.eval = rfx_host_eval;
    H.err = rfx_host_err;
    H.intern = rfx_host_intern;
    H.symname = rfx_host_symbol_name;
    H.null_obj = rfx_host_null();
    memset(H.f, 0, sizeof(H.f));
    H.bound = 2;
    return 0;
}

obj_p rfx_host_fn(const char *name) {
    static const struct { const char *n; int f; int type; int attrs; } T[] = {
        {"sum", F_SUM, RFX_TYPE_UNARY, RFX_FN_AGGR}, {"avg", F_AVG, RFX_TYPE_UNARY, RFX_FN_AGGR}, {"min", F_MIN, RFX_TYPE_UNARY, RFX_FN_AGGR},
        {"max", F_MAX, RFX_TYPE_UNARY, RFX_FN_AGGR}, {"count", F_COUNT, RFX_TYPE_UNARY, RFX_FN_AGGR}, {"first", F_FIRST, RFX_TYPE_UNARY, RFX_FN_AGGR},
        {"==", F_EQ, RFX_TYPE_BINARY, RFX_FN_ATOMIC}, {"!=", F_NE, RFX_TYPE_BINARY, RFX_FN_ATOMIC}, {"<", F_LT, RFX_TYPE_BINARY, RFX_FN_ATOMIC},
        {">", F_GT, RFX_TYPE_BINARY, RFX_FN_ATOMIC}, {"<=", F_LE, RFX_TYPE_BINARY, RFX_FN_ATOMIC}, {">=", F_GE, RFX_TYPE_BINARY, RFX_FN_ATOMIC},
        {"and", F_AND, RFX_TYPE_VARY, RFX_FN_SPECIAL_FORM}, {"or", F_OR, RFX_TYPE_VARY, RFX_FN_SPECIAL_FORM}, {"select", F_SELECT, RFX_TYPE_UNARY, 0},
        {"+", F_ADD, RFX_TYPE_BINARY, RFX_FN_ATOMIC}, {"-", F_SUB, RFX_TYPE_BINARY, RFX_FN_ATOMIC}, {"*", F_MUL, RFX_TYPE_BINARY, RFX_FN_ATOMIC},
        {"div", F_FDIV, RFX_TYPE_BINARY, RFX_FN_ATOMIC}, {"/", F_DIV, RFX_TYPE_BINARY, RFX_FN_ATOMIC}, {"%", F_MOD, RFX_TYPE_BINARY, RFX_FN_ATOMIC}, {"xbar", F_XBAR, RFX_TYPE_BINARY, RFX_FN_ATOMIC}, {"update", F_UPDATE, RFX_TYPE_UNARY, 0},
        {"med", F_MED, RFX_TYPE_UNARY, RFX_FN_AGGR}, {"dev", F_DEV, RFX_TYPE_UNARY, RFX_FN_AGGR},
        {"iasc", F_IASC, RFX_TYPE_UNARY, RFX_FN_NONE}, {"idesc", F_IDESC, RFX_TYPE_UNARY, RFX_FN_NONE}, {"asc", F_ASC, RFX_TYPE_UNARY, RFX_FN_NONE},
        {"desc", F_DESC, RFX_TYPE_UNARY, RFX_FN_NONE}, {"rank", F_RANK, RFX_TYPE_UNARY, RFX_FN_NONE}, {"xasc", F_XASC, RFX_TYPE_BINARY, RFX_FN_NONE},
        {"xdesc", F_XDESC, RFX_TYPE_BINARY, RFX_FN_NONE},
        {"asof-join", F_AJ, RFX_TYPE_VARY, RFX_FN_NONE}, {"bin", F_BIN, RFX_TYPE_BINARY, RFX_FN_NONE}, {"binr", F_BINR, RFX_TYPE_BINARY, RFX_FN_NONE},
        {"window-join", F_WJ, RFX_TYPE_VARY, RFX_FN_NONE}, {"window-join1", F_WJ1, RFX_TYPE_VARY, RFX_FN_NONE}, {"last", F_LAST, RFX_TYPE_UNARY, RFX_FN_AGGR},
        {"distinct", F_DISTINCT, RFX_TYPE_UNARY, RFX_FN_NONE}, {"find", F_FIND, RFX_TYPE_BINARY, RFX_FN_NONE}, {"in", F_IN, RFX_TYPE_BINARY, RFX_FN_NONE},
        {"sect", F_SECT, RFX_TYPE_BINARY, RFX_FN_NONE}, {"except", F_EXCEPT, RFX_TYPE_BINARY, RFX_FN_NONE}, {"union", F_UNION, RFX_TYPE_BINARY, RFX_FN_NONE},
        {"xrank", F_XRANK, RFX_TYPE_BINARY, RFX_FN_NONE}, {"floor", F_FLOOR, RFX_TYPE_UNARY, RFX_FN_ATOMIC}, {"ceil", F_CEIL, RFX_TYPE_UNARY, RFX_FN_ATOMIC},
        {"round", F_ROUND, RFX_TYPE_UNARY, RFX_FN_ATOMIC}, {"neg", F_NEG, RFX_TYPE_UNARY, RFX_FN_ATOMIC}};
    rfx_host_bind();
    for (size_t i = 0; i < sizeof(T) / sizeof(T[0]); i++)
        if (strcmp(T[i].n, name) == 0) {
            obj_p o = rfx_host_i64((int64_t)(intptr_t)OUR_FN[T[i].f]);
            o->type = (int8_t)T[i].type;
            o->attrs = (uint8_t)T[i].attrs;
            return o;
        }
    return NULL;
}

static obj_p fail(const char *msg) {
    rfx_host_bind();
    snprintf(g_err, sizeof(g_err), "%s", msg);
    return H.err(msg);
}
static obj_p fail_hip(const char *what) {
    char b[600];
    snprintf(b, sizeof(b), "%s: %s", what, rfx_hip_last_error());
    return fail(b);
}
static int g_refused_sharded;
static obj_p fail_ctx(void) {
    if (g_refused_sharded) return fail("this operator (or this shape of its arguments) needs its columns whole on one device: with RFX_SHARDS / RFX_DEVICES it is the host's own built-in -- joins, update, at over unordered ids, group over sparse keys, filtered MAPGROUP pairs");
    return fail_hip("no usable MI355X");
}
static obj_p refused1(int f, obj_p x);
__attribute__((unused)) static obj_p refused2(int f, obj_p x, obj_p y);
static obj_p refusedn(int f, obj_p *x, int64_t n);

static int fn_id(obj_p o) {
    if (!o || (o->type != RFX_TYPE_UNARY && o->type != RFX_TYPE_BINARY && o->type != RFX_TYPE_VARY)) return -1;
    void *p = (void *)(intptr_t)o->i64;
    for (int i = 0; i < F_N; i++)
        if ((OUR_FN[i] && p == OUR_FN[i]) || (H.f[i] && p == H.f[i])) return i;
    return -1;
}

#include "rfx_ops_residency.c"
#include "rfx_ops_repro.c"
#include "rfx_ops_plan.c"
#include "rfx_ops_select.c"
#include "rfx_ops_update.c"
#include "rfx_ops_operators.c"
#include "rfx_ops_join.c"
#include "rfx_ops_folds.c"
#include "rfx_ops_verbs.c"
#include "rfx_ops_sort.c"
#include "rfx_ops_asof.c"
#include "rfx_ops_window.c"
#include "rfx_ops_set.c"
#include "rfx_ops_bucket.c"
```

### rayforce_amd/csrc/rfx_ops_residency.c

```c
static rfx_ctx_t *g_ctx;
static rfx_ctx_t *g_ctxs[RFX_MAX_SHARDS];
static rfx_exec_t *g_x;
static int g_nshards = 1;
static int g_device = -1;
static int g_cfg_devices[RFX_MAX_SHARDS], g_cfg_ndev, g_cfg_shards;
int rfx_ops_set_device(int device) {
    if (g_ctx) return RFX_ESTATE;
    g_device = device;
    return RFX_OK;
}
int rfx_ops_set_shards(const int *devices, int ndevices, int nshards) {
    if (g_ctx) return RFX_ESTATE;
    if (ndevices < 0 || ndevices > RFX_MAX_SHARDS || nshards < 0 || nshards > RFX_MAX_SHARDS || (ndevices && !devices)) return RFX_EINVAL;
    for (int i = 0; i < ndevices; i++) g_cfg_devices[i] = devices[i];
    g_cfg_ndev = ndevices;
    g_cfg_shards = nshards;
    return RFX_OK;
}
int rfx_ops_shards(void) { return g_nshards; }
rfx_exec_t *rfx_ops_exec(void) { return g_x; }
static int ensure_ctx(void) {
    if (g_ctx) return RFX_OK;
    int devs[RFX_MAX_SHARDS], ndev = g_cfg_ndev, nsh = g_cfg_shards;
    for (int i = 0; i < ndev; i++) devs[i] = g_cfg_devices[i];
// ... 8 lines not shown
                while (*q && *q != ',') q++;
                if (*q == ',') q++;
            }
        }
    }
    if (ndev == 0) {
        if (g_device < 0) {
            const char *e = getenv("RFX_DEVICE");
            g_device = e ? atoi(e) : 0;
        }
        devs[ndev++] = g_device;
    }
    if (nsh == 0) {
        const char *e = getenv("RFX_SHARDS");
        nsh = e ? atoi(e) : 0;
    }
    if (nsh < ndev) nsh = ndev;
    if (nsh > RFX_MAX_SHARDS) nsh = RFX_MAX_SHARDS;
    int rc = RFX_OK, made = 0;
    for (int s = 0; s < nsh && rc == RFX_OK; s++) {
        rc = rfx_hip_ctx_create(devs[s % ndev], NULL, &g_ctxs[s]);
        if (rc == RFX_OK) made++;
    }
    if (rc == RFX_OK) rc = rfx_exec_create(g_ctxs, nsh, &g_x);
    if (rc == RFX_OK) rc = rfx_exec_comm_init_all(g_x);
    if (rc != RFX_OK) {
        if (g_x) rfx_exec_destroy(g_x);
        g_x = NULL;
        for (int s = 0; s < made; s++) { rfx_hip_ctx_destroy(g_ctxs[s]); g_ctxs[s] = NULL; }
        return rc;
    }
    g_device = devs[0];
    g_nshards = nsh;
    g_ctx = g_ctxs[0];
    rfx_hip_ctx_bind_thread(g_ctx);
    if (getenv("RFX_TRACE")) fprintf(stderr, "[rfx] operator layer: %d shard(s) over %d device(s)\n", nsh, ndev);
    return RFX_OK;
}
static void op_begin(void);
static void op_end(void);
int rfx_ops_dist_init(int world, int rank, const void *id128) {
    rfx_host_bind();
    op_begin();
    int rc = ensure_ctx();
    if (rc == RFX_OK && g_nshards > 1) rc = RFX_ESTATE;
    if (rc == RFX_OK) rc = rfx_dist_init(g_ctx, world, rank, id128);
    op_end();
    return rc;
}
int rfx_ops_dist_finalize(void) {
    if (!g_ctx) return RFX_OK;
    op_begin();
    const int rc = rfx_dist_finalize(g_ctx);
    op_end();
    return rc;
}
__attribute__((unused)) static int ensure_ctx1(void) {
    const int rc = ensure_ctx();
    g_refused_sharded = rc == RFX_OK && g_nshards > 1;
    return g_refused_sharded ? RFX_ELIMIT : rc;
}

typedef struct {
    const void *host;
    int64_t len;
    int type;
    uint64_t sum;
    void *dev;
    size_t bytes;
    int pinned;
    uint64_t tick, epoch;
    int tracked;
    int stable;
    int sd_never;
    uint64_t edge_sum;
    size_t dbytes;
    int scope_ok;
    int64_t smin, smax;
    void *devs[RFX_MAX_SHARDS];
    obj_p owner;
    int amax_ok;
    double amax;
    int fix_k, fix_m;
} resident_t;
static resident_t *g_res;
static int g_nres, g_capres;
static uint64_t g_tick, g_epoch = 1;
static size_t g_res_bytes;
static int64_t g_stat[10];
static int64_t g_sd_hits;
static int64_t g_sum_validations;
static int64_t g_own_hits;
static int64_t g_own_released;
static int64_t g_fix_built, g_fix_hits;
static int g_validate = -1;
static int validate_mode(void) {
    if (g_validate < 0) {
        const char *e = getenv("RFX_VALIDATE");
        g_validate = (e && (strcmp(e, "checksum") == 0 || strcmp(e, "1") == 0)) ? 1 : 0;
    }
    return g_validate;
}
static inline uint32_t obj_rc(obj_p o) { return __atomic_load_n(&o->rc, __ATOMIC_RELAXED); }
enum { ST_SELECT_GPU, ST_SELECT_DELEGATED, ST_JOIN_GPU, ST_JOIN_DELEGATED, ST_UPLOADS, ST_CACHE_HITS, ST_CACHE_STALE, ST_OPS, ST_SCOPE_SAMPLED, ST_SCOPE_RETRIED };

typedef struct {
    const unsigned char *p;
    size_t bytes;
    uint64_t h;
} sum_job_t;
#define SUM_ROTL(x, r) (((x) << (r)) | ((x) >> (64 - (r))))
static uint64_t sum_range(const unsigned char *p, size_t bytes) {
    const uint64_t K = 0x9E3779B97F4A7C15ULL;
    uint64_t h0 = 0x243F6A8885A308D3ULL, h1 = 0x13198A2E03707344ULL, h2 = 0xA4093822299F31D0ULL, h3 = 0x082EFA98EC4E6C89ULL;
    size_t nw = bytes / 8, i = 0;
    const uint64_t *w = (const uint64_t *)p;
    if (((uintptr_t)p & 7) == 0) {
        for (; i + 4 <= nw; i += 4) {
            h0 = SUM_ROTL(h0 ^ w[i], 31) * K;
            h1 = SUM_ROTL(h1 ^ w[i + 1], 31) * K;
            h2 = SUM_ROTL(h2 ^ w[i + 2], 31) * K;
            h3 = SUM_ROTL(h3 ^ w[i + 3], 31) * K;
        }
        for (; i < nw; i++) h0 = SUM_ROTL(h0 ^ w[i], 31) * K;
    } else i = 0, nw = 0;
    uint64_t h = (SUM_ROTL(h0 ^ (h1 >> 29), 31) * K) ^ (SUM_ROTL(h2 ^ (h3 >> 31) ^ (h1 << 35) ^ (h3 << 33), 27) * K);
    for (size_t b = nw * 8; b < bytes; b++) h = SUM_ROTL(h ^ p[b], 31) * K;
    return h ^ (h >> 32);
}
static void *sum_worker(void *arg) {
    sum_job_t *j = (sum_job_t *)arg;
    j->h = sum_range(j->p, j->bytes);
    return NULL;
}
static uint64_t payload_sum(const void *p, size_t bytes) {
    enum { MAXT = 32 };
    int nt = 1;
    if (bytes >= ((size_t)8 << 20)) {
        long cores = sysconf(_SC_NPROCESSORS_ONLN);
        nt = cores > MAXT ? MAXT : (cores < 1 ? 1 : (int)cores);
        if ((size_t)nt > bytes >> 22) nt = (int)(bytes >> 22);
    }
    if (nt <= 1) return sum_range((const unsigned char *)p, bytes) ^ (uint64_t)bytes;
    sum_job_t job[MAXT];
    pthread_t th[MAXT];
    size_t per = ((bytes / (size_t)nt) + 63) & ~(size_t)63, off = 0;
    int started = 0;
    for (int i = 0; i < nt; i++) {
        job[i].p = (const unsigned char *)p + off;
        job[i].bytes = (i == nt - 1 || off + per > bytes) ? bytes - off : per;
        off += job[i].bytes;
        if (i < nt - 1 && pthread_create(&th[i], NULL, sum_worker, &job[i]) == 0) started |= 1 << i;
        else sum_worker(&job[i]);
    }
    uint64_t h = (uint64_t)bytes;
    for (int i = 0; i < nt; i++) {
        if (started & (1 << i)) pthread_join(th[i], NULL);
        h = SUM_ROTL(h ^ job[i].h, 31) * 0x9E3779B97F4A7C15ULL;
    }
    return h;
}

#define SD_MIN_BYTES ((size_t)1 << 20)
#define SD_STABLE_USES 2
static int g_sd_state = -1;
static int g_sd_pagemap = -1;
// ... 569 lines not shown
```

### rayforce_amd/csrc/rfx_ops_select.c

```c
static double g_tm[12];
static int g_ntm;
static void tm_mark(void) {
    if (g_ntm < 12) {
        struct timespec ts;
        clock_gettime(CLOCK_MONOTONIC, &ts);
        g_tm[g_ntm++] = ts.tv_sec * 1e6 + ts.tv_nsec * 1e-3;
    }
}
static void tm_print(void) {
    static int on = -1;
    if (on < 0) { const char *e = getenv("RFX_TRACE"); on = e && atoi(e) >= 2; }
    if (on && g_ntm > 1) {
        fprintf(stderr, "[rfx] select us:");
        for (int i = 1; i < g_ntm; i++) fprintf(stderr, " %.0f", g_tm[i] - g_tm[i - 1]);
        fprintf(stderr, "  (plan | scope | tables+pass+rank | emit | fetch | build+free) total %.0f\n", g_tm[g_ntm - 1] - g_tm[0]);
    }
}
enum { SEL_GO = 0, SEL_OUT = 1, SEL_DONE = 2 };
#define SEL_AGGS (2 * RFX_MAX_AGGS + 1)
typedef struct {
    rfx_agg_t aggs[SEL_AGGS];
    rfx_xnode_t xnodes[RFX_MAX_AGGS][RFX_MAX_XNODES];
    int64_t names[RFX_MAX_AGGS];
    int outtype[RFX_MAX_AGGS];
// ... 547 lines not shown
            if (parted) { why = "med over a parted table"; goto out; }
            if (g_nshards > 1) { why = "med over a sharded table"; goto out; }
            if (rfx_exec_ranks(g_x, NULL) > 1) { why = "med over several ranks"; goto out; }
        }
        if (M.ndev) {
            if (where) { why = "dev under where: (ray_dev of a MAPFILTER pair answers null in the reference)"; goto out; }
            if (parted) { why = "dev over a parted table"; goto out; }
            if (g_nshards > 1) { why = "dev over a sharded table"; goto out; }
            if (rfx_exec_ranks(g_x, NULL) > 1) { why = "dev over several ranks"; goto out; }
        }
        if (M.nlast) {
            if (parted) { why = "last over a parted table"; goto out; }
            if (rfx_exec_ranks(g_x, NULL) > 1) { why = "last over several ranks"; goto out; }
        }
        obj_p kcs[RFX_MAX_KEYS] = {0};
        const void *dks[RFX_MAX_KEYS] = {0};
        int64_t knames[RFX_MAX_KEYS], kxbar[RFX_MAX_KEYS] = {0};
        int nkeys = 0;
        int8_t key_out_type = RFX_TYPE_I64;
        obj_p kenum = NULL;
        if (by) {
            if (sel_by_shape(tab, by, kcs, knames, kxbar, &nkeys, &why) == SEL_OUT) goto out;
            for (int i = 0; i < nkeys; i++) {
                if (parted) {
                    const proxy_t *px = kcs[i] ? proxy_of(kcs[i]) : NULL;
                    if (nkeys != 1 || !px || px->kind != 2 || kcs[i]->type != RFX_TYPE_I64) { why = "parted table: by: is not the virtual column"; goto out; }
                    key_out_type = px->vtype;
                } else if (kcs[i] && kcs[i]->type == RFX_TYPE_ENUM && nkeys == 1 && !kxbar[i]) {
                    kenum = kcs[i];
                    if (resident(enum_indices(kcs[i]), 0, &dks[i]) != RFX_OK) { res = fail_hip("column upload"); goto done; }
                    key_out_type = RFX_TYPE_SYMBOL;
                    continue;
                }
                const int f64key = kcs[i] && kcs[i]->type == RFX_TYPE_F64 && nkeys == 1 && !kxbar[i] && !parted;
                if (!kcs[i] || !(kcs[i]->type == RFX_TYPE_I64 || kcs[i]->type == RFX_TYPE_SYMBOL || kcs[i]->type == RFX_TYPE_TIMESTAMP || f64key)) {
                    why = "by: key is not an 8-byte integer column";
                    goto out;
                }
                if (kxbar[i] > 0 && kcs[i]->type == RFX_TYPE_SYMBOL) { why = "xbar over a symbol column"; goto out; }
                if (nkeys == 1 && !parted) key_out_type = kcs[i]->type;
                if (resident(kcs[i], 0, &dks[i]) != RFX_OK) { res = fail_hip("column upload"); goto done; }
            }
            if (nkeys > 1 && where) { why = "where: with several by: columns"; goto out; }
        }
        rfx_query_t Q;
        memset(&Q, 0, sizeof(Q));
        Q.preds = wp.preds;
        Q.npred = wp.npred;
        Q.logic = wp.logic;
        Q.aggs = M.aggs;
        Q.nagg = M.nagg;
        Q.nkeys = nkeys;
        Q.d_keys = dks;
        Q.kxbar = kxbar;
        Q.nrows = nrows;
        if (!flat && g_nshards > 1) {
            const void *mcol = NULL;
            const int mrc = mask_column_sharded(tab, where, nrows, &mcol);
            if (mrc == -1) { why = "where: shape"; goto out; }
            if (mrc) { res = fail_hip("where"); goto done; }
            memset(&wp.preds[0], 0, sizeof(wp.preds[0]));
            wp.preds[0].d_col = mcol;
            wp.preds[0].col_type = RFX_I64;
            wp.preds[0].op = RFX_NE;
            wp.preds[0].rhs_type = RFX_I64;
            wp.preds[0].rhs_i = 0;
            wp.npred = 1;
            wp.logic = RFX_AND;
            Q.preds = wp.preds;
            Q.npred = 1;
            Q.logic = RFX_AND;
        } else if (!flat) {
            int8_t *m = NULL;
            const int mrc = mask_of_expr(tab, where, nrows, &m);
            if (mrc == -1) { why = "where: shape"; goto out; }
            if (mrc) { res = fail_hip("where"); goto done; }
            tmp[ntmp++] = m;
            Q.d_mask = m;
        }
        if (by && !parted && det_mode()) {
            if (det_rewrite(&M, nrows) != 0) { res = fail_hip("deterministic sums"); goto done; }
            Q.nagg = M.nagg + M.nhidden;
        }
        Q.cols = g_nshards > 1 ? g_qcols : NULL;
        Q.ncols = g_nqcols;
        tm_mark();
        if (!by && M.nagg == 0) {
            if (sel_projection(tab, &Q, parted, &res, &why) == SEL_OUT) goto out;
            goto done;
        }
        if (by) {
            int64_t kscope[2];
            Q.flags = RFX_Q_REFUSE_NULL_KEY |
                      RFX_Q_SLICED;
            resident_t *ke = (g_nshards == 1 && nkeys == 1 && !parted && flat && nrows > 0 && nrows < ((int64_t)1 << 24) && !kxbar[0]) ? resident_entry(dks[0]) : NULL;
            if (ke) {
                if (!ke->scope_ok) {
                    int64_t c0 = 0;
                    if (rfx_hip_scope_i64(g_ctx, (const int64_t *)dks[0], NULL, 0, RFX_AND, nrows, &ke->smin, &ke->smax, &c0) != RFX_OK) { res = fail_hip("scope"); goto done; }
                    ke->scope_ok = 1;
                }
                kscope[0] = ke->smin;
                kscope[1] = ke->smax;
                Q.key_scope = kscope;
            }
            rfx_groups_t R;
            const int grc = rfx_exec_group_by(g_x, &Q, &R);
            tm_mark();
            if (grc == RFX_EXEC_NULL_KEY) { why = "null group key"; goto out; }
            if (grc == RFX_ESTATE && strstr(rfx_exec_last_error(g_x), "collision")) { why = "row-hash collision between two key tuples"; goto out; }
            if (grc == RFX_ELIMIT && g_nshards > 1) { why = M.nlast ? "sharded table: last under by: runs on the shards of one device" : "sharded table: shape the planner runs on one shard"; goto out; }
            if (grc != RFX_OK) { res = fail(rfx_exec_last_error(g_x)); goto done; }
            const sel_keys_t K = {nkeys, key_out_type, kenum, kcs};
            rfx_groups_t Rw;
            const rfx_groups_t *Ru = &R;
            if (rank_slices_mode()) {
                int rank = 0;
                const int ranks = rfx_exec_ranks(g_x, &rank);
                int64_t g0 = 0, gn = R.groups;
                if (ranks > 1) rfx_exec_split(R.groups, ranks, rank, &g0, &gn);
                if (ranks > 1 && rfx_exec_groups_window(&R, g0, gn, &Rw) == RFX_OK) Ru = &Rw;
            }
            res = sel_build_groups(Ru, &M, &K, knames, &why);
            rfx_exec_groups_free(g_x, &R);
            tm_mark();
            if (!res) goto out;
            g_last_gpu = res->type == RFX_TYPE_TABLE;
            goto done;
        }
        rfx_value_t vals[RFX_MAX_AGGS];
        int64_t selected = 0;
        if (rfx_exec_filter_aggr(g_x, &Q, vals, &selected) != RFX_OK) { res = fail(rfx_exec_last_error(g_x)); goto done; }
        for (int a = 0; a < M.nagg; a++) {
            if (!M.med[a]) continue;
            const int mrc = rfx_exec_median(g_x, &Q, M.aggs[a].d_col, M.aggs[a].col_type, &vals[a]);
            if (mrc == RFX_ENOMEM) { why = "med: device scratch (8 B per row) not available"; goto out; }
            if (mrc != RFX_OK) { res = fail(rfx_exec_last_error(g_x)); goto done; }
        }
        for (int a = 0; a < M.nagg; a++) {
            if (!M.dev[a]) continue;
            const int drc = rfx_exec_dev(g_x, &Q, M.aggs[a].d_col, M.aggs[a].col_type, &vals[a]);
            if (drc == RFX_ENOMEM) { why = "dev: device scratch not available"; goto out; }
            if (drc != RFX_OK) { res = fail(rfx_exec_last_error(g_x)); goto done; }
        }
        res = sel_build_scalar(vals, &M);
        g_last_gpu = 1;
        goto done;
    }
out:
    for (int i = 0; i < ntmp; i++) rfx_hip_free(g_ctx, tmp[i]);
    ntmp = 0;
    qtmp_release();
    if (parted) parted_view_release();
    parted = 0;
    res = delegate_select(dict, why ? why : "unsupported");
done:
    for (int i = 0; i < ntmp; i++) rfx_hip_free(g_ctx, tmp[i]);
    qtmp_release();
    if (parted) parted_view_release();
    H.drop(host_tab);
    tm_mark();
    tm_print();
    if (take && g_last_gpu && res && res->type == RFX_TYPE_TABLE) {
        obj_p tv = HOST_CALL(H.eval(take));
        if (tv && tv->type != RFX_TYPE_ERR) {
            obj_p cut = HOST_CALL(((rfx_binary_f)H.f[F_TAKE])(res, tv));
            H.drop(res);
            res = cut;
        } else {
            H.drop(res);
            res = tv;
        }
        if (tv && res != tv) H.drop(tv);
    }
    return res;
}
rfx_obj_p rfx_select(rfx_obj_p dict) {
    op_begin();
    g_last_gpu = 0;
    obj_p r = select_impl(dict);
    g_stat[g_last_gpu ? ST_SELECT_GPU : ST_SELECT_DELEGATED]++;
    op_end();
    return r;
}
```

### rayforce_amd/engine.py

```python
from __future__ import annotations

import ctypes as C
from typing import Dict, List, Optional, Sequence, Tuple, Union

import torch

from . import _lib as L
from . import marshal as M
from ._lib import RfxError
from .marshal import NotFused as _NotFused, ctype_of as _ctype_of

Column = torch.Tensor


class _Owner:

    def __init__(self, eng, struct, free):
        self.eng, self.struct, self.free = eng, struct, free

    def __del__(self):
        try:
            if self.eng._x:
                self.free(self.eng._x, C.byref(self.struct))
        except Exception:
            pass


class _View:
    def __init__(self, owner, ptr: int, n: int, typestr: str):
        self.owner = owner
        self.__cuda_array_interface__ = {"shape": (int(n),), "typestr": typestr, "data": (int(ptr), False), "version": 2}


class Engine:

    def __init__(self, device: Union[int, torch.device, None] = None, shards: int = 1):
        self.lib = L.load_library()
        if not torch.cuda.is_available():
            raise RfxError("no GPU visible to torch: the MI355X engine has no CPU fallback")
        if device is None:
            device = torch.cuda.current_device()
        self.device = torch.device("cuda", device if isinstance(device, int) else device.index)
        torch.cuda.set_device(self.device)
        self.shards = int(shards)
        self._ctxs = (C.c_void_p * self.shards)()
        stream = torch.cuda.current_stream(self.device).cuda_stream or 1
        for s in range(self.shards):
            c = C.c_void_p()
            L.check(self.lib.rfx_hip_ctx_create(self.device.index, C.c_void_p(stream if s == 0 else 0), C.byref(c)), "ctx_create")
            self._ctxs[s] = c.value
        self._ctx = C.c_void_p(self._ctxs[0])
        self._x = C.c_void_p()
        L.check(self.lib.rfx_exec_create(self._ctxs, self.shards, C.byref(self._x)), "exec_create")
        self._keep: List = []
        self.last_set_route = "none"

    def close(self) -> None:
        if self._x:
            self.lib.rfx_exec_destroy(self._x)
            self._x = C.c_void_p()
            for s in range(self.shards):
                self.lib.rfx_hip_ctx_destroy(C.c_void_p(self._ctxs[s]))
            self._ctx = C.c_void_p()

    def __del__(self):
        try:
            self.close()
        except Exception:
            pass

    def _xcheck(self, rc: int, what: str) -> None:
        if rc != L.RFX_OK:
            raise RfxError(f"{what} failed with code {rc}: {self.lib.rfx_exec_last_error(self._x).decode(errors='replace')}")

    def sync(self) -> None:
        L.check(self.lib.rfx_hip_ctx_sync(self._ctx), "sync")

    def trim(self) -> None:
        for s in range(self.shards):
            L.check(self.lib.rfx_hip_ctx_trim(C.c_void_p(self._ctxs[s])), "ctx_trim")

    def tune(self, blocks_per_cu: int = 0, flags: int = 0) -> None:
        for s in range(self.shards):
            L.check(self.lib.rfx_hip_ctx_tune(C.c_void_p(self._ctxs[s]), blocks_per_cu, flags), "tune")

    def stat(self, which: int) -> int:
        return sum(int(self.lib.rfx_hip_ctx_stat(C.c_void_p(self._ctxs[s]), which)) for s in range(self.shards))

    def xstat(self, which: int) -> int:
        return int(self.lib.rfx_exec_stat(self._x, which))

    @property
    def spec_retries(self) -> int:
        return self.xstat(L.RFX_XSTAT_SCOPE_RETRIED)

    def forget_scopes(self) -> None:
        self.lib.rfx_exec_forget_scopes(self._x)

    def timer_start(self) -> None:
        L.check(self.lib.rfx_hip_timer_start(self._ctx), "timer_start")

    def timer_stop(self) -> float:
        ms = C.c_float()
        L.check(self.lib.rfx_hip_timer_stop(self._ctx, C.byref(ms)), "timer_stop")
        return float(ms.value)

    def profile(self, enable: bool = True) -> None:
        L.check(self.lib.rfx_hip_ctx_profile(self._ctx, int(enable)), "ctx_profile")

    def last_kernel_ms(self) -> float:
        ms = C.c_float()
        L.check(self.lib.rfx_hip_last_kernel_ms(self._ctx, C.byref(ms)), "last_kernel_ms")
        return float(ms.value)

    def empty(self, n: int, dtype=torch.int64) -> torch.Tensor:
        return torch.empty(int(n), dtype=dtype, device=self.device)

    def column(self, host_array) -> torch.Tensor:
        t = torch.as_tensor(host_array)
        if t.dtype not in (torch.int64, torch.float64, torch.int8, torch.bool):
            raise RfxError(f"unsupported dtype {t.dtype}")
        return (t.to(torch.int8) if t.dtype == torch.bool else t).contiguous().to(self.device)

    def upload(self, host_array) -> torch.Tensor:
        import numpy as np
        a = np.ascontiguousarray(host_array)
        if a.ndim != 1 or a.dtype not in (np.int64, np.float64):
            raise RfxError(f"upload: a 1-d int64 / float64 array is expected, not {a.dtype} with shape {a.shape}")
        out = torch.empty(a.shape[0], dtype=torch.float64 if a.dtype == np.float64 else torch.int64, device=self.device)
        L.check(self.lib.rfx_hip_h2d_pipelined(self._ctx, out.data_ptr(), a.ctypes.data, a.nbytes), "h2d_pipelined")
        return out

    def gen_i64(self, n: int, seed: int, modulus: int, row0: int = 0, out: Optional[torch.Tensor] = None) -> torch.Tensor:
        out = self.empty(n, torch.int64) if out is None else out
        L.check(self.lib.rfx_hip_gen_i64(self._ctx, out.data_ptr(), n, seed, row0, modulus), "gen_i64")
        return out

    def gen_f64(self, n: int, seed: int, row0: int = 0, out: Optional[torch.Tensor] = None) -> torch.Tensor:
        out = self.empty(n, torch.float64) if out is None else out
        L.check(self.lib.rfx_hip_gen_f64(self._ctx, out.data_ptr(), n, seed, row0), "gen_f64")
        return out

    def load_column(self, path: str) -> torch.Tensor:
        from . import colfiles
        return colfiles.load_column(self, path)

    def load_splayed(self, directory: str, columns: Optional[Sequence[str]] = None) -> Dict[str, torch.Tensor]:
        from . import colfiles
        return colfiles.load_splayed(self, directory, columns)

    def load_parted(self, root: str, table: str, columns: Optional[Sequence[str]] = None, where=None) -> Dict[str, torch.Tensor]:
        from . import colfiles
        return colfiles.load_parted(self, root, table, columns, where)

    def _check_col(self, t, n=None):
        return M.check_col(self, t, n)

    def _resolve(self, x, table):
        return M.resolve(self, x, table)

    def _query(self, where, aggs, table, nrows: Optional[int], keys=None, flags: int = 0) -> Tuple[L.Query, int]:
        self._keep.clear()
        q = L.Query()
        n = nrows
        if isinstance(where, torch.Tensor):
            m = self._check_col(where.view(torch.int8) if where.dtype == torch.bool else where, n)
            if m.dtype != torch.int8:
                raise RfxError("where expects a B8 mask")
            q.d_mask, n = m.data_ptr(), m.numel()
            self._keep.append(m)
        else:
            try:
                logic, leaves, more = M.tree_leaves(self, where)
            except _NotFused:
                return self._query(self.mask_of(where, table), aggs, table, nrows, keys, flags)
            parr, n = M.preds(self, leaves, more, table, n)
            q.preds, q.npred, q.logic = parr, len(leaves), logic
            self._keep.append(parr)
        aarr, n = M.aggs(self, aggs or [], table, n)
        q.aggs, q.nagg = aarr, len(aggs or [])
        self._keep.append(aarr)
        if keys:
            kx = (C.c_int64 * len(keys))()
            kp = (C.c_void_p * len(keys))()
            for i, k in enumerate(keys):
                if isinstance(k, tuple) and len(k) == 3 and k[0] == "xbar":
                    if int(k[2]) <= 0:
                        raise RfxError("xbar: width must be positive")
                    col, kx[i] = self._check_col(self._resolve(k[1], table), n), int(k[2])
                else:
                    col = self._check_col(self._resolve(k, table), n)
                if col.dtype != torch.int64:
                    raise RfxError("group key must be i64 on this path (f64 keys group on their bit pattern: view as int64)")
                n = col.numel() if n is None else n
                kp[i] = col.data_ptr()
                self._keep.append(col)
# ... 387 lines not shown
```

### rayforce_amd/hostobj.py

```python
from __future__ import annotations

import ctypes as C
from typing import Dict, Sequence

import numpy as np

from . import _lib as L

T_LIST, T_B8, T_I64, T_SYMBOL, T_F64, T_TABLE, T_DICT, T_ERR = 0, 1, 5, 6, 10, 98, 99, 127
NP_OF = {T_B8: np.int8, T_I64: np.int64, T_SYMBOL: np.int64, T_F64: np.float64, 9: np.int64, 4: np.int32, 7: np.int32, 8: np.int32}
TYPE_OF = {np.dtype(np.int8): T_B8, np.dtype(np.bool_): T_B8, np.dtype(np.int64): T_I64, np.dtype(np.float64): T_F64}

OPS_PROTOTYPES = {
    "rfx_host_bind": (C.c_int, []),
    "rfx_ops_set_device": (C.c_int, [C.c_int]),
    "rfx_ops_last_error": (C.c_char_p, []),
    "rfx_ops_set_shards": (C.c_int, [C.POINTER(C.c_int), C.c_int, C.c_int]),
    "rfx_ops_shards": (C.c_int, []),
    "rfx_ops_set_validation": (C.c_int, [C.c_int]),
    "rfx_ops_set_deterministic": (C.c_int, [C.c_int]),
    "rfx_ops_set_rank_slices": (C.c_int, [C.c_int]),
    "rfx_ops_dist_init": (C.c_int, [C.c_int, C.c_int, C.c_void_p]),
    "rfx_ops_dist_finalize": (C.c_int, []),
    "rfx_ops_exec": (C.c_void_p, []),
    "rfx_host_device_vector": (C.c_void_p, [C.c_int8, C.c_int64, C.POINTER(C.c_void_p), C.c_int]),
    "rfx_select": (C.c_void_p, [C.c_void_p]),
    "rfx_update": (C.c_void_p, [C.c_void_p]),
    **{f"rfx_{n}": (C.c_void_p, [C.c_void_p, C.c_void_p]) for n in ("eq", "ne", "lt", "gt", "le", "ge", "at", "add", "sub", "mul", "div", "floordiv", "mod")},
    "rfx_and": (C.c_void_p, [C.POINTER(C.c_void_p), C.c_int64]),
    "rfx_or": (C.c_void_p, [C.POINTER(C.c_void_p), C.c_int64]),
    "rfx_and_sf": (C.c_void_p, [C.POINTER(C.c_void_p), C.c_int64]),
    "rfx_or_sf": (C.c_void_p, [C.POINTER(C.c_void_p), C.c_int64]),
    "rfx_left_join": (C.c_void_p, [C.POINTER(C.c_void_p), C.c_int64]),
    "rfx_inner_join": (C.c_void_p, [C.POINTER(C.c_void_p), C.c_int64]),
    **{f"rfx_{n}": (C.c_void_p, [C.c_void_p]) for n in ("where", "sum", "avg", "min", "max", "count", "first", "last", "dev", "pin", "unpin", "invalidate", "stats", "group", "med", "iasc", "idesc", "asc", "desc", "rank")},
    "rfx_xasc": (C.c_void_p, [C.c_void_p, C.c_void_p]),
    "rfx_xdesc": (C.c_void_p, [C.c_void_p, C.c_void_p]),
    "rfx_last_sort_on_gpu": (C.c_int, []),
    "rfx_asof_join": (C.c_void_p, [C.POINTER(C.c_void_p), C.c_int64]),
    "rfx_bin": (C.c_void_p, [C.c_void_p, C.c_void_p]),
    "rfx_binr": (C.c_void_p, [C.c_void_p, C.c_void_p]),
    "rfx_last_asof_on_gpu": (C.c_int, []),
    "rfx_window_join": (C.c_void_p, [C.POINTER(C.c_void_p), C.c_int64]),
    "rfx_window_join1": (C.c_void_p, [C.POINTER(C.c_void_p), C.c_int64]),
    "rfx_last_window_on_gpu": (C.c_int, []),
    "rfx_distinct": (C.c_void_p, [C.c_void_p]),
    **{f"rfx_{n}": (C.c_void_p, [C.c_void_p, C.c_void_p]) for n in ("find", "in", "sect", "except", "union")},
    "rfx_last_set_on_gpu": (C.c_int, []),
    "rfx_last_set_route": (C.c_int, []),
    "rfx_set_stats": (C.c_void_p, [C.c_void_p]),
    **{f"rfx_{n}": (C.c_void_p, [C.c_void_p, C.c_void_p]) for n in ("xrank", "xbar", "within")},
    **{f"rfx_{n}": (C.c_void_p, [C.c_void_p]) for n in ("floor", "ceil", "round", "neg")},
    "rfx_last_bucket_on_gpu": (C.c_int, []),
    "rfx_cache_clear": (None, []),
    "rfx_cache_bytes": (C.c_int64, []),
    "rfx_last_select_on_gpu": (C.c_int, []),
    "rfx_host_vector": (C.c_void_p, [C.c_int8, C.c_int64]),
    "rfx_host_i64": (C.c_void_p, [C.c_int64]),
    "rfx_host_f64": (C.c_void_p, [C.c_double]),
    "rfx_host_symbol": (C.c_void_p, [C.c_char_p]),
    "rfx_host_list": (C.c_void_p, [C.c_int64]),
    "rfx_host_table": (C.c_void_p, [C.c_void_p, C.c_void_p]),
    "rfx_host_dict": (C.c_void_p, [C.c_void_p, C.c_void_p]),
    "rfx_host_fn": (C.c_void_p, [C.c_char_p]),
    "rfx_host_clone": (C.c_void_p, [C.c_void_p]),
    "rfx_host_drop": (None, [C.c_void_p]),
    "rfx_host_intern": (C.c_int64, [C.c_char_p, C.c_int64]),
    "rfx_host_symbol_name": (C.c_char_p, [C.c_int64]),
    "rfx_host_error_text": (C.c_char_p, [C.c_void_p]),
}


class Header(C.Structure):
    _fields_ = [("mmod", C.c_uint8), ("order", C.c_uint8), ("type", C.c_int8), ("attrs", C.c_uint8), ("rc", C.c_uint32), ("len", C.c_int64)]


_bound = None


def lib() -> C.CDLL:
    global _bound
    if _bound is None:
        l = L.load_library()
        for name, (res, args) in OPS_PROTOTYPES.items():
            fn = getattr(l, name)
            fn.restype, fn.argtypes = res, args
        _bound = l
    return _bound


def header(o: int) -> Header:
    return Header.from_address(o)


def payload(o: int) -> int:
    return o + 16


def vector(a: np.ndarray) -> int:
    a = np.ascontiguousarray(a)
    t = TYPE_OF[a.dtype]
    o = lib().rfx_host_vector(t, a.size)
    if a.size:
        C.memmove(payload(o), a.ctypes.data, a.nbytes)
    return o


def to_numpy(o: int) -> np.ndarray:
    h = header(o)
    dt = NP_OF[h.type]
    return np.frombuffer((C.c_char * (h.len * np.dtype(dt).itemsize)).from_address(payload(o)), dtype=dt).copy() if h.len else np.empty(0, dt)


def list_of(items: Sequence[int]) -> int:
    o = lib().rfx_host_list(len(items))
    arr = (C.c_void_p * len(items)).from_address(payload(o))
    for i, it in enumerate(items):
        arr[i] = it
# ... 74 lines not shown
```

Baseline: 203.0 billion.

## Add cached 4-byte images of i64 key/predicate columns for plane scatter group-by

Builds and caches an int32 copy of i64 key and predicate columns when all values fit, registers the copies as aliases per context, and has the plane scatter kernel read 4-byte elements for those columns through templated narrow loads. This halves HBM traffic for the key and predicate columns of a single-key, single-value group-by. In exchange it adds a one-time narrowing pass, extra device memory held in the residency cache, more kernel template instances, and alias bookkeeping that must be cleared after each query.

```diff
diff --git a/include/rfx_hip.h b/include/rfx_hip.h
--- a/include/rfx_hip.h
+++ b/include/rfx_hip.h
@@ -159,7 +159,10 @@
     RFX_STAT_CHUNK_SCATTER = 3,
     RFX_STAT_CHUNK_AGGREGATE = 4,
     RFX_STAT_MASK_PASSES = 5,
-    RFX_STAT_WHERE_ONCE = 6
+    RFX_STAT_WHERE_ONCE = 6,
+    RFX_STAT_PLANE_NARROW = 7,
+    RFX_STAT_PLANE_LAST_NW = 8,
+    RFX_STAT_PLANE_LAST_PBITS = 9
 };
 int64_t rfx_hip_ctx_stat(rfx_ctx_t *ctx, int which);
 
@@ -181,6 +184,9 @@
 int rfx_column_file_stat(const char *path, int32_t *type, int64_t *len);
 int rfx_hip_column_file_load(rfx_ctx_t *ctx, const char *path, void *d_dst, int64_t nrows);
 int rfx_hip_widen_i32(rfx_ctx_t *ctx, const int32_t *d_in, int64_t n, int64_t *d_out);
+int rfx_hip_narrow_i64(rfx_ctx_t *ctx, const int64_t *d_in, int64_t n, int32_t *d_out, int *fits);
+int rfx_hip_ctx_narrow_alias(rfx_ctx_t *ctx, const void *d_col8, const int32_t *d_col4, int64_t nrows);
+int rfx_hip_ctx_narrow_clear(rfx_ctx_t *ctx);
 int rfx_hip_widen_b8(rfx_ctx_t *ctx, const int8_t *d_in, int64_t n, int64_t *d_out);
 
 int rfx_hip_timer_start(rfx_ctx_t *ctx);
diff --git a/include/rfx_ops.h b/include/rfx_ops.h
--- a/include/rfx_ops.h
+++ b/include/rfx_ops.h
@@ -99,6 +99,7 @@
 int rfx_ops_set_deterministic(int mode);
 int rfx_ops_set_rank_slices(int on);
 rfx_obj_p rfx_stats(rfx_obj_p ignored);
+rfx_obj_p rfx_narrow_stats(rfx_obj_p ignored);
 void rfx_cache_clear(void);
 int64_t rfx_cache_bytes(void);
 int rfx_last_select_on_gpu(void);
diff --git a/rayforce_amd/_lib.py b/rayforce_amd/_lib.py
--- a/rayforce_amd/_lib.py
+++ b/rayforce_amd/_lib.py
@@ -220,6 +220,9 @@
     "rfx_hip_where_begin": (C.c_int, [_ctx, _P(Pred), C.c_int, C.c_int, C.c_void_p, C.c_int64, _P(C.c_int64)]),
     "rfx_hip_where_emit": (C.c_int, [_ctx, C.c_int64, C.c_void_p]),
     "rfx_hip_widen_i32": (C.c_int, [_ctx, C.c_void_p, C.c_int64, C.c_void_p]),
+    "rfx_hip_narrow_i64": (C.c_int, [_ctx, C.c_void_p, C.c_int64, C.c_void_p, _P(C.c_int)]),
+    "rfx_hip_ctx_narrow_alias": (C.c_int, [_ctx, C.c_void_p, C.c_void_p, C.c_int64]),
+    "rfx_hip_ctx_narrow_clear": (C.c_int, [_ctx]),
     "rfx_hip_widen_b8": (C.c_int, [_ctx, C.c_void_p, C.c_int64, C.c_void_p]),
     "rfx_hip_where_estimate": (C.c_int, [_ctx, _P(Pred), C.c_int, C.c_int, C.c_int64, _P(C.c_int64)]),
     "rfx_hip_where_once": (C.c_int, [_ctx, _P(Pred), C.c_int, C.c_int, C.c_int64, C.c_int64, C.c_void_p, C.c_int64, _P(C.c_int64)]),
diff --git a/rayforce_amd/csrc/rfx_ctx.hip b/rayforce_amd/csrc/rfx_ctx.hip
--- a/rayforce_amd/csrc/rfx_ctx.hip
+++ b/rayforce_amd/csrc/rfx_ctx.hip
@@ -63,6 +63,7 @@
 static void pool_release(rfx_ctx *c);
 void rfx_plane_release(rfx_ctx *c);
 void rfx_plane_invalidate(rfx_ctx *c);
+i64 rfx_plane_stat(rfx_ctx *c, int which);
 extern "C" int rfx_hip_ctx_destroy(rfx_ctx_t *c) {
     if (!c) return RFX_OK;
     (void)hipSetDevice(c->device);
@@ -99,7 +100,8 @@
 }
 
 extern "C" int64_t rfx_hip_ctx_stat(rfx_ctx_t *c, int which) {
-    if (!c || which < 0 || which > 6) return -1;
+    if (!c || which < 0 || which > RFX_STAT_PLANE_LAST_PBITS) return -1;
+    if (which >= RFX_STAT_PLANE_NARROW && which <= RFX_STAT_PLANE_LAST_PBITS) return (int64_t)rfx_plane_stat(c, which);
     if (which == 6) return (int64_t)(uintptr_t)c->ext_p[4];
     return which == RFX_STAT_MASK_PASSES ? c->ext_i[0] : c->ext_i[3 + which];
 }
diff --git a/rayforce_amd/csrc/rfx_group_plane.hip b/rayforce_amd/csrc/rfx_group_plane.hip
--- a/rayforce_amd/csrc/rfx_group_plane.hip
+++ b/rayforce_amd/csrc/rfx_group_plane.hip
@@ -11,6 +11,7 @@
 #define PL_QFLUSH 24
 #define PL_SPIN_LIMIT (1u << 14)
 #define PL_MAX_NV 3
+#define PL_MAX_ALIAS 64
 #ifndef PL_META64_PLAIN
 #define PL_META64_PLAIN 1
 #endif
@@ -41,7 +42,13 @@
 #define PL_LD(ptr) __hip_atomic_load((ptr), __ATOMIC_RELAXED, __HIP_MEMORY_SCOPE_WORKGROUP)
 #define PL_ST(ptr, v) __hip_atomic_store((ptr), (v), __ATOMIC_RELAXED, __HIP_MEMORY_SCOPE_WORKGROUP)
 
-template <int NC, int NP, int NV, int PBITS, int VGL, bool HK = false>
+typedef int pl_i2 __attribute__((ext_vector_type(2)));
+__device__ __forceinline__ void pl_ld2n(const u64 *col32, i64 row, u64 &a, u64 &b) {
+    const pl_i2 t = __builtin_nontemporal_load((const pl_i2 *)((const int *)col32 + row));
+    a = (u64)(i64)t.x;
+    b = (u64)(i64)t.y;
+}
+template <int NC, int NP, int NV, int PBITS, int VGL, bool HK = false, unsigned NW = 0u>
 __global__ __launch_bounds__(PL_T) void k_plane_scatter(const Plan P, const PlaneArgs A) {
     constexpr int PARTS = pl_parts<PBITS, VGL, HK>();
     constexpr bool P192 = PARTS != (1 << PBITS);
@@ -208,6 +215,10 @@
                 for (int c = 0; c < NC; c++) {
 #pragma unroll
                     for (int j = 0; j < 4; j++) {
+                        if ((NW >> c) & 1u) {
+                            pl_ld2n(P.cols[c], base + j * 128, va[c][2 * j], va[c][2 * j + 1]);
+                            continue;
+                        }
                         const u64x2 t = rfx_ld2(P.cols[c] + base + j * 128);
                         va[c][2 * j] = t.x;
                         va[c][2 * j + 1] = t.y;
@@ -220,6 +231,10 @@
                     if ((A.pmask >> c) & 1u) {
 #pragma unroll
                         for (int j = 0; j < 4; j++) {
+                            if ((NW >> c) & 1u) {
+                                pl_ld2n(P.cols[c], base + j * 128, va[c][2 * j], va[c][2 * j + 1]);
+                                continue;
+                            }
                             const u64x2 t = rfx_ld2(P.cols[c] + base + j * 128);
                             va[c][2 * j] = t.x;
                             va[c][2 * j + 1] = t.y;
@@ -236,6 +251,10 @@
 #pragma unroll
                         for (int j = 0; j < 4; j++) {
                             if ((m >> (2 * j)) & 3u) {
+                                if ((NW >> c) & 1u) {
+                                    pl_ld2n(P.cols[c], base + j * 128, va[c][2 * j], va[c][2 * j + 1]);
+                                    continue;
+                                }
                                 const u64x2 t = rfx_ld2(P.cols[c] + base + j * 128);
                                 va[c][2 * j] = t.x;
                                 va[c][2 * j + 1] = t.y;
@@ -257,7 +276,7 @@
             const bool in = row < r1;
             valid |= (unsigned)in << e;
 #pragma unroll
-            for (int c = 0; c < NC; c++) va[c][e] = in ? P.cols[c][row] : 0ULL;
+            for (int c = 0; c < NC; c++) va[c][e] = !in ? 0ULL : (((NW >> c) & 1u) ? (u64)(i64)((const int *)P.cols[c])[row] : P.cols[c][row]);
         }
         step(va, (NP == 0) ? valid : eval_preds<NC, 8, NP>(S, va, valid), base);
     }
@@ -508,32 +527,57 @@
     for (int j = 0; j < nv; j++) A->vals[j] = (u64 *)(w + o_val + plane * j);
 }
 
-template <int NC, int NP, int NV, int PBITS, int VGL, bool HK = false>
+template <int NC, int NP, int NV, int PBITS, int VGL, bool HK = false, unsigned NW = 0u>
 static int launch_plane_scatter_inst(rfx_ctx *c, const Plan &P, const PlaneArgs &A) {
     constexpr size_t lds = pl_lds_bytes<NV, PBITS, VGL, HK>();
     static_assert(lds <= 160 * 1024, "rings beyond a CU's LDS");
     static unsigned long long attr_set = 0;
     if (!((attr_set >> (c->device & 63)) & 1ull)) {
-        RFX_HIP_CHECK(hipFuncSetAttribute((const void *)k_plane_scatter<NC, NP, NV, PBITS, VGL, HK>, hipFuncAttributeMaxDynamicSharedMemorySize, (int)lds));
+        RFX_HIP_CHECK(hipFuncSetAttribute((const void *)k_plane_scatter<NC, NP, NV, PBITS, VGL, HK, NW>, hipFuncAttributeMaxDynamicSharedMemorySize, (int)lds));
         __atomic_fetch_or(&attr_set, 1ull << (c->device & 63), __ATOMIC_RELAXED);
     }
-    hipLaunchKernelGGL((k_plane_scatter<NC, NP, NV, PBITS, VGL, HK>), dim3(A.nblk), dim3(PL_T), lds, c->stream, P, A);
+    hipLaunchKernelGGL((k_plane_scatter<NC, NP, NV, PBITS, VGL, HK, NW>), dim3(A.nblk), dim3(PL_T), lds, c->stream, P, A);
     return RFX_OK;
 }
-template <int NC, int NV, int PBITS, int VGL, bool HK = false>
+template <int NC, int NV, int PBITS, int VGL, bool HK = false, unsigned NW = 0u>
 static int launch_plane_scatter_np(rfx_ctx *c, const Plan &P, const PlaneArgs &A) {
-    if (P.npred == 0) return launch_plane_scatter_inst<NC, 0, NV, PBITS, VGL, HK>(c, P, A);
-    if (P.npred == 1) return launch_plane_scatter_inst<NC, 1, NV, PBITS, VGL, HK>(c, P, A);
-    if (P.npred <= 3) return launch_plane_scatter_inst<NC, 3, NV, PBITS, VGL, HK>(c, P, A);
-    return launch_plane_scatter_inst<NC, RFX_MAX_PREDS, NV, PBITS, VGL, HK>(c, P, A);
-}
-static int launch_plane_scatter(rfx_ctx *c, const Plan &P, const PlaneArgs &A, int pbits) {
+    if constexpr (NW != 0u) {
+        if constexpr (NC == 1 + NV) {
+            if (P.npred == 0) return launch_plane_scatter_inst<NC, 0, NV, PBITS, VGL, HK, NW>(c, P, A);
+        }
+        if (P.npred == 1) return launch_plane_scatter_inst<NC, 1, NV, PBITS, VGL, HK, NW>(c, P, A);
+        return RFX_ESTATE;
+    } else {
+        if (P.npred == 0) return launch_plane_scatter_inst<NC, 0, NV, PBITS, VGL, HK, NW>(c, P, A);
+        if (P.npred == 1) return launch_plane_scatter_inst<NC, 1, NV, PBITS, VGL, HK, NW>(c, P, A);
+        if (P.npred <= 3) return launch_plane_scatter_inst<NC, 3, NV, PBITS, VGL, HK, NW>(c, P, A);
+        return launch_plane_scatter_inst<NC, RFX_MAX_PREDS, NV, PBITS, VGL, HK, NW>(c, P, A);
+    }
+}
+static bool plane_narrow_form(const Plan &Pc, int nv) { return nv == 1 && (Pc.npred == 1 || (Pc.npred == 0 && Pc.ncols == 1 + nv)); }
+template <int PBITS, int VGL>
+static int launch_plane_scatter_nv1(rfx_ctx *c, const Plan &P, const PlaneArgs &A, int extra, unsigned nw) {
+    if (extra == 0) {
+        if (nw == 0u) return launch_plane_scatter_np<2, 1, PBITS, VGL>(c, P, A);
+        if (nw == 1u) return launch_plane_scatter_np<2, 1, PBITS, VGL, false, 1u>(c, P, A);
+    } else if (extra == 1) {
+        if (nw == 0u) return launch_plane_scatter_np<3, 1, PBITS, VGL>(c, P, A);
+        if (nw == 1u) return launch_plane_scatter_np<3, 1, PBITS, VGL, false, 1u>(c, P, A);
+        if (nw == 4u) return launch_plane_scatter_np<3, 1, PBITS, VGL, false, 4u>(c, P, A);
+        if (nw == 5u) return launch_plane_scatter_np<3, 1, PBITS, VGL, false, 5u>(c, P, A);
+    } else {
+        if (nw == 0u) return launch_plane_scatter_np<4, 1, PBITS, VGL>(c, P, A);
+        if (nw == 1u) return launch_plane_scatter_np<4, 1, PBITS, VGL, false, 1u>(c, P, A);
+        if (nw == 12u) return launch_plane_scatter_np<4, 1, PBITS, VGL, false, 12u>(c, P, A);
+        if (nw == 13u) return launch_plane_scatter_np<4, 1, PBITS, VGL, false, 13u>(c, P, A);
+    }
+    return RFX_ESTATE;
+}
+static int launch_plane_scatter(rfx_ctx *c, const Plan &P, const PlaneArgs &A, int pbits, unsigned nw) {
     const int extra = P.ncols - 1 - A.nv;
     if (extra < 0 || extra > 2) return RFX_ESTATE;
-    if (A.nv == 1) {
-        if (pbits == 7) return extra == 0 ? launch_plane_scatter_np<2, 1, 7, 5>(c, P, A) : (extra == 1 ? launch_plane_scatter_np<3, 1, 7, 5>(c, P, A) : launch_plane_scatter_np<4, 1, 7, 5>(c, P, A));
-        return extra == 0 ? launch_plane_scatter_np<2, 1, 8, 4>(c, P, A) : (extra == 1 ? launch_plane_scatter_np<3, 1, 8, 4>(c, P, A) : launch_plane_scatter_np<4, 1, 8, 4>(c, P, A));
-    }
+    if (A.nv == 1) return pbits == 7 ? launch_plane_scatter_nv1<7, 5>(c, P, A, extra, nw) : launch_plane_scatter_nv1<8, 4>(c, P, A, extra, nw);
+    if (nw != 0u) return RFX_ESTATE;
     if (pbits != 7 || extra > 1) return RFX_ESTATE;
     if (A.nv == 2) return extra == 0 ? launch_plane_scatter_np<3, 2, 7, 4>(c, P, A) : launch_plane_scatter_np<4, 2, 7, 4>(c, P, A);
     return extra == 0 ? launch_plane_scatter_np<4, 3, 7, 4>(c, P, A) : launch_plane_scatter_np<5, 3, 7, 4>(c, P, A);
@@ -580,17 +624,54 @@
     i64 nrows;
     i64 seen;
     u64 sig[RFX_MAX_PREDS][6];
+    i64 narrow_launches;
+    unsigned last_nw;
+    int last_pbits;
+    int nalias;
+    struct { const void *col8; const int *col4; i64 nrows; } alias[PL_MAX_ALIAS];
 };
 static PlaneState *plane_state(rfx_ctx *c) {
     if (!c->ext_p[2]) c->ext_p[2] = calloc(1, sizeof(PlaneState));
     return (PlaneState *)c->ext_p[2];
 }
+i64 rfx_plane_stat(rfx_ctx *c, int which) {
+    const PlaneState *st = (const PlaneState *)c->ext_p[2];
+    if (!st) return 0;
+    return which == RFX_STAT_PLANE_NARROW ? st->narrow_launches : (which == RFX_STAT_PLANE_LAST_NW ? (i64)st->last_nw : (i64)st->last_pbits);
+}
 void rfx_plane_invalidate(rfx_ctx *c) {
     if (c->ext_p[2]) ((PlaneState *)c->ext_p[2])->valid = 0;
 }
 void rfx_plane_release(rfx_ctx *c) {
     free(c->ext_p[2]);
     c->ext_p[2] = NULL;
+}
+extern "C" int rfx_hip_ctx_narrow_alias(rfx_ctx_t *c, const void *d_col8, const int32_t *d_col4, int64_t nrows) {
+    RFX_REQUIRE(c && d_col8 && d_col4 && nrows > 0, RFX_EINVAL, "narrow_alias: NULL argument / no rows");
+    RFX_REQUIRE(((uintptr_t)d_col4 & 7u) == 0, RFX_EINVAL, "narrow_alias: the image is not 8-byte aligned");
+    PlaneState *st = plane_state(c);
+    RFX_REQUIRE(st != NULL, RFX_ENOMEM, "host calloc failed");
+    int at = st->nalias;
+    for (int i = 0; i < st->nalias; i++)
+        if (st->alias[i].col8 == d_col8) at = i;
+    RFX_REQUIRE(at < PL_MAX_ALIAS, RFX_ELIMIT, "narrow_alias: table full");
+    st->alias[at].col8 = d_col8;
+    st->alias[at].col4 = (const int *)d_col4;
+    st->alias[at].nrows = (i64)nrows;
+    if (at == st->nalias) st->nalias++;
+    return RFX_OK;
+}
+extern "C" int rfx_hip_ctx_narrow_clear(rfx_ctx_t *c) {
+    RFX_REQUIRE(c, RFX_EINVAL, "ctx is NULL");
+    if (c->ext_p[2]) ((PlaneState *)c->ext_p[2])->nalias = 0;
+    return RFX_OK;
+}
+static const int *plane_alias(const PlaneState *st, const void *col, i64 nrows) {
+    static const char *off = getenv("RFX_NO_NARROW");
+    if (off && atoi(off) != 0) return NULL;
+    for (int i = 0; i < st->nalias; i++)
+        if (st->alias[i].col8 == col && st->alias[i].nrows == nrows) return st->alias[i].col4;
+    return NULL;
 }
 static void plane_pred_sig(const Plan &P, u64 (*sig)[6]) {
     for (int i = 0; i < P.npred; i++) {
@@ -665,12 +746,32 @@
         if (Pc.preds[i].rhs_col >= 0) A.pmask |= 1u << Pc.preds[i].rhs_col;
     }
     if (getenv("RFX_PLANE_LOAD_ALL")) A.pmask = 0xFFu;
+    unsigned nw = 0;
+    if (st->nalias > 0 && plane_narrow_form(Pc, nv)) {
+        const int *k4 = plane_alias(st, (const void *)Pc.cols[0], nrows), *e4[2] = {NULL, NULL};
+        bool ext = Pc.ncols > 2 && Pc.npred > 0;
+        for (int i = 2; i < Pc.ncols; i++) {
+            e4[i - 2] = plane_alias(st, (const void *)Pc.cols[i], nrows);
+            if (!e4[i - 2]) ext = false;
+        }
+        if (k4) {
+            nw |= 1u;
+            Pc.cols[0] = (const u64 *)k4;
+        }
+        for (int i = 2; ext && i < Pc.ncols; i++) {
+            nw |= 1u << i;
+            Pc.cols[i] = (const u64 *)e4[i - 2];
+        }
+    }
     RFX_HIP_CHECK(hipMemsetAsync(A.ctl, 0, 256, c->stream));
     c->ext_i[3 + RFX_STAT_PLANE_SCATTER]++;
     RFX_KERNEL_BEGIN(c);
-    int rc = launch_plane_scatter(c, Pc, A, pbits);
+    int rc = launch_plane_scatter(c, Pc, A, pbits, nw);
     RFX_KERNEL_END(c);
     if (rc != RFX_OK) return rc;
+    st->last_nw = nw;
+    st->last_pbits = pbits;
+    if (nw) st->narrow_launches++;
     RFX_HIP_CHECK(hipGetLastError());
     unsigned *hctl = (unsigned *)c->h_pin;
     RFX_HIP_CHECK(hipMemcpyAsync(hctl, A.ctl, 256, hipMemcpyDeviceToHost, c->stream));
diff --git a/rayforce_amd/csrc/rfx_io.hip b/rayforce_amd/csrc/rfx_io.hip
--- a/rayforce_amd/csrc/rfx_io.hip
+++ b/rayforce_amd/csrc/rfx_io.hip
@@ -306,6 +306,50 @@
         out[i] = x == (int32_t)0x80000000 ? (long long)0x8000000000000000ULL : (long long)x;
     }
 }
+template <bool VEC>
+__global__ __launch_bounds__(256) void k_narrow_i64(const long long *__restrict__ in, long long n, int *__restrict__ out, unsigned *__restrict__ bad) {
+    typedef long long l2 __attribute__((ext_vector_type(2)));
+    typedef int i2 __attribute__((ext_vector_type(2)));
+    bool b = false;
+    auto fits = [](long long x) { return x >= -2147483647LL && x <= 2147483647LL; };
+    const long long pairs = VEC ? n >> 1 : 0;
+    for (long long p = blockIdx.x * 256LL + threadIdx.x; p < pairs; p += (long long)gridDim.x * 256LL) {
+        const l2 t = __builtin_nontemporal_load((const l2 *)in + p);
+        b = b || !fits(t.x) || !fits(t.y);
+        i2 o;
+        o.x = (int)t.x;
+        o.y = (int)t.y;
+        ((i2 *)out)[p] = o;
+    }
+    for (long long i = 2 * pairs + blockIdx.x * 256LL + threadIdx.x; i < n; i += (long long)gridDim.x * 256LL) {
+        const long long x = in[i];
+        b = b || !fits(x);
+        out[i] = (int)x;
+    }
+    if (__any(b) && (threadIdx.x & 63) == 0) atomicOr(bad, 1u);
+}
+extern "C" int rfx_hip_narrow_i64(rfx_ctx_t *c, const int64_t *d_in, int64_t n, int32_t *d_out, int *fits) {
+    RFX_REQUIRE(c && fits, RFX_EINVAL, "NULL argument");
+    *fits = 1;
+    if (n <= 0) return RFX_OK;
+    RFX_REQUIRE(d_in && d_out, RFX_EINVAL, "NULL argument");
+    int rc = rfx_ws_reserve(c, 256);
+    if (rc != RFX_OK) return rc;
+    unsigned *bad = (unsigned *)c->d_ws;
+    RFX_HIP_CHECK(hipMemsetAsync(bad, 0, 4, c->stream));
+    const bool vec = (((uintptr_t)d_in & 15u) | ((uintptr_t)d_out & 7u)) == 0;
+    long long blocks = ((vec ? (n + 1) / 2 : n) + 255) / 256;
+    int grid = c->num_cus * 16;
+    if (blocks < grid) grid = (int)blocks;
+    if (vec) hipLaunchKernelGGL(k_narrow_i64<true>, dim3(grid), dim3(256), 0, c->stream, (const long long *)d_in, (long long)n, (int *)d_out, bad);
+    else hipLaunchKernelGGL(k_narrow_i64<false>, dim3(grid), dim3(256), 0, c->stream, (const long long *)d_in, (long long)n, (int *)d_out, bad);
+    RFX_HIP_CHECK(hipGetLastError());
+    unsigned *h = (unsigned *)c->h_pin;
+    RFX_HIP_CHECK(hipMemcpyAsync(h, bad, 4, hipMemcpyDeviceToHost, c->stream));
+    RFX_HIP_CHECK(hipStreamSynchronize(c->stream));
+    *fits = h[0] == 0;
+    return RFX_OK;
+}
 __global__ __launch_bounds__(256) void k_widen_b8(const int8_t *__restrict__ in, long long n, long long *__restrict__ out) {
     for (long long i = blockIdx.x * 256LL + threadIdx.x; i < n; i += (long long)gridDim.x * 256LL) out[i] = in[i] ? 1LL : 0LL;
 }
diff --git a/rayforce_amd/csrc/rfx_ops.c b/rayforce_amd/csrc/rfx_ops.c
--- a/rayforce_amd/csrc/rfx_ops.c
+++ b/rayforce_amd/csrc/rfx_ops.c
@@ -169,6 +169,7 @@
 
 #include "rfx_ops_residency.c"
 #include "rfx_ops_repro.c"
+#include "rfx_ops_narrow.c"
 #include "rfx_ops_plan.c"
 #include "rfx_ops_select.c"
 #include "rfx_ops_update.c"
diff --git a/rayforce_amd/csrc/rfx_ops_narrow.c b/rayforce_amd/csrc/rfx_ops_narrow.c
--- /dev/null
+++ b/rayforce_amd/csrc/rfx_ops_narrow.c
@@ -0,0 +1,92 @@
+#define NARROW_TYPE(t) ((t) + 768)
+static int64_t g_nw_built, g_nw_hits, g_nw_refused;
+static int narrow_off(void) {
+    static int off = -1;
+    if (off < 0) {
+        const char *e = getenv("RFX_NO_NARROW");
+        off = e && atoi(e) != 0;
+    }
+    return off;
+}
+static int resident_narrow(const void *base_dev, int64_t nrows, void **devs_out ) {
+    resident_t *re = resident_entry(base_dev);
+    if (!re || !re->owner || validate_mode() != 0 || re->len != nrows || nrows <= 0) return 1;
+    if (!(re->type == RFX_TYPE_I64 || re->type == RFX_TYPE_TIMESTAMP || re->type == RFX_TYPE_SYMBOL) || re->narrow_no) return 1;
+    const int itype = NARROW_TYPE(re->type);
+    for (int i = 0; i < g_nres; i++) {
+        if (g_res[i].owner != re->owner || g_res[i].type != itype) continue;
+        if (g_res[i].len != nrows) { res_free(i); break; }
+        g_res[i].tick = ++g_tick;
+        g_res[i].epoch = g_epoch;
+        g_nw_hits++;
+        for (int s = 0; s < RFX_MAX_SHARDS; s++) devs_out[s] = g_res[i].devs[s];
+        return RFX_OK;
+    }
+    re = resident_entry(base_dev);
+    if (!re) return 1;
+    const resident_t base = *re;
+    res_make_room((size_t)nrows * 4);
+    if (g_res_bytes + (size_t)nrows * 4 > cache_budget()) return 1;
+    void *devs[RFX_MAX_SHARDS];
+    int rc = shards_alloc(devs, nrows, 4, 0), fits = 1;
+    if (rc != RFX_OK) return rc == RFX_ENOMEM ? 1 : rc;
+    for (int s = 0; s < g_nshards && rc == RFX_OK && fits; s++) {
+        int64_t n;
+        rfx_exec_split(nrows, g_nshards, s, NULL, &n);
+        if (g_nshards == 1) n = nrows;
+        if (n <= 0) continue;
+        if (g_nshards > 1) rfx_hip_ctx_bind_thread(g_ctxs[s]);
+        rc = rfx_hip_narrow_i64(g_ctxs[s], (const int64_t *)base.devs[s], n, (int32_t *)devs[s], &fits);
+    }
+    if (rc != RFX_OK || !fits) {
+        for (int s = 0; s < g_nshards; s++) { if (g_nshards > 1) rfx_hip_ctx_bind_thread(g_ctxs[s]); rfx_hip_free(g_ctxs[s], devs[s]); }
+        if (g_nshards > 1) rfx_hip_ctx_bind_thread(g_ctx);
+        if (rc != RFX_OK) return rc;
+        re = resident_entry(base_dev);
+        if (re) re->narrow_no = 1;
+        g_nw_refused++;
+        return 1;
+    }
+    if (g_nshards > 1) rfx_hip_ctx_bind_thread(g_ctx);
+    resident_t e;
+    memset(&e, 0, sizeof(e));
+    e.host = base.host; e.len = nrows; e.type = itype; e.dev = devs[0]; e.bytes = base.bytes; e.tick = ++g_tick; e.epoch = g_epoch; e.dbytes = (size_t)nrows * 4;
+    e.owner = H.clone(base.owner);
+    for (int s = 0; s < g_nshards; s++) e.devs[s] = devs[s];
+    res_append(&e);
+    g_nw_built++;
+    for (int s = 0; s < RFX_MAX_SHARDS; s++) devs_out[s] = s < g_nshards ? devs[s] : NULL;
+    return RFX_OK;
+}
+static int g_narrow_told;
+static void narrow_forget(void) {
+    if (!g_narrow_told) return;
+    for (int s = 0; s < g_nshards; s++) rfx_hip_ctx_narrow_clear(g_ctxs[s]);
+    g_narrow_told = 0;
+}
+static int narrow_tell(const void *base_dev, int64_t nrows) {
+    void *img[RFX_MAX_SHARDS];
+    const int rc = resident_narrow(base_dev, nrows, img);
+    if (rc != RFX_OK) return rc == 1 ? RFX_OK : rc;
+    const resident_t *re = resident_entry(base_dev);
+    if (!re) return RFX_OK;
+    for (int s = 0; s < g_nshards; s++) {
+        int64_t n;
+        rfx_exec_split(nrows, g_nshards, s, NULL, &n);
+        if (g_nshards == 1) n = nrows;
+        if (n <= 0 || !img[s] || !re->devs[s]) continue;
+        if (rfx_hip_ctx_narrow_alias(g_ctxs[s], re->devs[s], (const int32_t *)img[s], n) == RFX_OK) g_narrow_told = 1;
+    }
+    return RFX_OK;
+}
+rfx_obj_p rfx_narrow_stats(rfx_obj_p x) {
+    (void)x;
+    rfx_host_bind();
+    op_begin();
+    obj_p out = H.vector(RFX_TYPE_I64, 3);
+    RFX_AS_I64(out)[0] = g_nw_built;
+    RFX_AS_I64(out)[1] = g_nw_hits;
+    RFX_AS_I64(out)[2] = g_nw_refused;
+    op_end();
+    return out;
+}
diff --git a/rayforce_amd/csrc/rfx_ops_residency.c b/rayforce_amd/csrc/rfx_ops_residency.c
--- a/rayforce_amd/csrc/rfx_ops_residency.c
+++ b/rayforce_amd/csrc/rfx_ops_residency.c
@@ -114,6 +114,7 @@
     int amax_ok;
     double amax;
     int fix_k, fix_m;
+    int narrow_no;
 } resident_t;
 static resident_t *g_res;
 static int g_nres, g_capres;
diff --git a/rayforce_amd/csrc/rfx_ops_select.c b/rayforce_amd/csrc/rfx_ops_select.c
--- a/rayforce_amd/csrc/rfx_ops_select.c
+++ b/rayforce_amd/csrc/rfx_ops_select.c
@@ -653,6 +653,30 @@
             if (det_rewrite(&M, nrows) != 0) { res = fail_hip("deterministic sums"); goto done; }
             Q.nagg = M.nagg + M.nhidden;
         }
+        if (by && nkeys == 1 && !parted && flat && !kxbar[0] && !narrow_off() && validate_mode() == 0 && nrows / g_nshards >= ((int64_t)1 << 22)) {
+            const void *vcols[SEL_AGGS], *told[1 + 2 * RFX_MAX_PREDS];
+            int nv = 0, plain = 1, ntold = 0;
+            for (int a = 0; a < Q.nagg && plain; a++) {
+                const rfx_agg_t *ag = &M.aggs[a];
+                if (ag->nxnodes > 0 || ag->xop != RFX_X_NONE) plain = 0;
+                if (ag->kind == RFX_AGG_COUNT || ag->kind == RFX_AGG_FIRST || !ag->d_col) continue;
+                int j = 0;
+                while (j < nv && vcols[j] != ag->d_col) j++;
+                if (j == nv) vcols[nv++] = ag->d_col;
+            }
+            if (plain && nv == 1) {
+                told[ntold++] = dks[0];
+                for (int i = 0; i < Q.npred; i++) {
+                    if (Q.preds[i].col_type == RFX_I64 && Q.preds[i].d_col) told[ntold++] = Q.preds[i].d_col;
+                    if (Q.preds[i].rhs_type == RFX_I64 && Q.preds[i].d_rhs_col) told[ntold++] = Q.preds[i].d_rhs_col;
+                }
+                for (int i = 0; i < ntold; i++) {
+                    int seen = 0;
+                    for (int j = 0; j < i; j++) seen |= told[j] == told[i];
+                    if (!seen && narrow_tell(told[i], nrows) != RFX_OK) { res = fail_hip("4-byte column image"); goto done; }
+                }
+            }
+        }
         Q.cols = g_nshards > 1 ? g_qcols : NULL;
         Q.ncols = g_nqcols;
         tm_mark();
@@ -721,12 +745,14 @@
 out:
     for (int i = 0; i < ntmp; i++) rfx_hip_free(g_ctx, tmp[i]);
     ntmp = 0;
+    narrow_forget();
     qtmp_release();
     if (parted) parted_view_release();
     parted = 0;
     res = delegate_select(dict, why ? why : "unsupported");
 done:
     for (int i = 0; i < ntmp; i++) rfx_hip_free(g_ctx, tmp[i]);
+    narrow_forget();
     qtmp_release();
     if (parted) parted_view_release();
     H.drop(host_tab);
diff --git a/rayforce_amd/engine.py b/rayforce_amd/engine.py
--- a/rayforce_amd/engine.py
+++ b/rayforce_amd/engine.py
@@ -53,6 +53,7 @@
         self._x = C.c_void_p()
         L.check(self.lib.rfx_exec_create(self._ctxs, self.shards, C.byref(self._x)), "exec_create")
         self._keep: List = []
+        self._narrow: List = []
         self.last_set_route = "none"
 
     def close(self) -> None:
@@ -112,6 +113,22 @@
         ms = C.c_float()
         L.check(self.lib.rfx_hip_last_kernel_ms(self._ctx, C.byref(ms)), "last_kernel_ms")
         return float(ms.value)
+
+    def narrow(self, col: torch.Tensor) -> Optional[torch.Tensor]:
+        if self.shards != 1 or col.dtype != torch.int64 or not col.is_contiguous() or col.numel() == 0:
+            raise RfxError("narrow: a non-empty contiguous int64 column on a one-shard engine is expected")
+        img = torch.empty(col.numel(), dtype=torch.int32, device=self.device)
+        fits = C.c_int()
+        L.check(self.lib.rfx_hip_narrow_i64(self._ctx, col.data_ptr(), col.numel(), img.data_ptr(), C.byref(fits)), "narrow_i64")
+        if not fits.value:
+            return None
+        L.check(self.lib.rfx_hip_ctx_narrow_alias(self._ctx, col.data_ptr(), img.data_ptr(), col.numel()), "narrow_alias")
+        self._narrow.append((col, img))
+        return img
+
+    def narrow_clear(self) -> None:
+        L.check(self.lib.rfx_hip_ctx_narrow_clear(self._ctx), "narrow_clear")
+        self._narrow.clear()
 
     def empty(self, n: int, dtype=torch.int64) -> torch.Tensor:
         return torch.empty(int(n), dtype=dtype, device=self.device)
diff --git a/rayforce_amd/hostobj.py b/rayforce_amd/hostobj.py
--- a/rayforce_amd/hostobj.py
+++ b/rayforce_amd/hostobj.py
@@ -33,7 +33,7 @@
     "rfx_or_sf": (C.c_void_p, [C.POINTER(C.c_void_p), C.c_int64]),
     "rfx_left_join": (C.c_void_p, [C.POINTER(C.c_void_p), C.c_int64]),
     "rfx_inner_join": (C.c_void_p, [C.POINTER(C.c_void_p), C.c_int64]),
-    **{f"rfx_{n}": (C.c_void_p, [C.c_void_p]) for n in ("where", "sum", "avg", "min", "max", "count", "first", "last", "dev", "pin", "unpin", "invalidate", "stats", "group", "med", "iasc", "idesc", "asc", "desc", "rank")},
+    **{f"rfx_{n}": (C.c_void_p, [C.c_void_p]) for n in ("where", "sum", "avg", "min", "max", "count", "first", "last", "dev", "pin", "unpin", "invalidate", "stats", "narrow_stats", "group", "med", "iasc", "idesc", "asc", "desc", "rank")},
     "rfx_xasc": (C.c_void_p, [C.c_void_p, C.c_void_p]),
     "rfx_xdesc": (C.c_void_p, [C.c_void_p, C.c_void_p]),
     "rfx_last_sort_on_gpu": (C.c_int, []),
```

After: 215.6 billion, median of 6. 6.2% higher.
